# migoox/genome-downsampler

Measured on AMD Instinct MI355X. Metric: Mreads/s selected at target coverage M=100, higher is better.
Workload: dtype u32

## Files before the change

genome-downsampler_amd/csrc/api/context.inc.hip:

```cpp
namespace {

thread_local char g_err[512] = "";

int fail(int code, const char* fmt, ...) {
    va_list ap;
    va_start(ap, fmt);
    vsnprintf(g_err, sizeof(g_err), fmt, ap);
    va_end(ap);
    return code;
}

#define HIP_TRY(expr)                                                                      \
    do {                                                                                   \
        hipError_t _e = (expr);                                                            \
        if (_e != hipSuccess)                                                              \
            return fail(_e == hipErrorOutOfMemory ? QMCP_ENOMEM : QMCP_EHIP, "%s: %s (%s:%d)", \
                        #expr, hipGetErrorString(_e), __FILE__, __LINE__);                 \
    } while (0)

struct DevBuf {
    void* p = nullptr;
    size_t cap = 0;
};

enum Ev { EV_BEGIN = 0, EV_PREP, EV_SCAN, EV_SORT, EV_SWEEP, EV_MARK, EV_COUNT };

struct Problem {
    uint64_t n = 0;
    uint32_t n_contigs = 0;
    uint64_t ltot = 0;
    std::vector<uint64_t> poff;
};

struct SolveRun {
    const uint32_t* d_starts = nullptr;
    const uint32_t* d_ends = nullptr;
    const uint64_t* roff = nullptr;
    const uint32_t* lengths = nullptr;
    uint32_t n_contigs = 0, M = 0;
    uint64_t n64 = 0;
    uint64_t* d_mask = nullptr;
    Problem pr;
    qmcp_hip_stats local;
    bool trivial = false, head_done = false, may_rank = false, two_level = false, have_gstart = true;
    bool ranked_counted = false, wait_empty = false;
    bool pm = false;
    uint32_t range_shift = 0;
    uint32_t nu_filter = 0;
};

}

struct qmcp_hip_ctx {
    int device = 0;
    qmcp_hip_options opt = {};
    hipStream_t stream = nullptr;
    hipEvent_t ev[EV_COUNT] = {};
    hipEvent_t ev_in = nullptr;
    hipStream_t stream2 = nullptr;
    hipEvent_t ev_fork = nullptr;
    DevBuf roff, poff, stats, cstart, boff, ecnt, eoff, selend, spine, hist, spine2, hist2, specsnap, specflags;
    DevBuf keys[2], vals[2];
    DevBuf in_starts, in_ends, in_aux0, in_aux1, mask, cov, amp, next_head;
    DevBuf f_starts, f_ends, f_map, f_words, f_mask;
    DevBuf ranges;
    DevBuf rankamb;
    DevBuf pm_desc, pm_work;
    uint32_t nu_ell = 0;
    uint64_t nu_failed_n = 0, nu_failed_ltot = 0;
    uint32_t nu_failed_ell = 0, nu_failed_M = 0;
    uint64_t nu_need_n = 0, nu_need_ltot = 0;
    uint32_t nu_need_ell = 0, nu_need_M = 0, nu_need_rounds = 0;
    bool nu_deferred = false;
    DevBuf nu_exc, nu_nadj, nu_ce, nu_state, nu_sus, nu_ckpt, nu_prev;
    uint32_t* h_nu = nullptr;
    uint64_t* h_tables = nullptr;
    size_t h_tables_cap = 0;
    unsigned long long* h_scalars = nullptr;
    uint32_t* h_stage = nullptr;
    size_t h_stage_words = 0;
    uint64_t* h_mask = nullptr;
    size_t h_mask_words = 0;
    std::vector<hipEvent_t> stage_ev;
    std::vector<hipStream_t> stage_streams;
    std::vector<hipEvent_t> stage_done;
    bool pending = false;
    qmcp_hip_stats pend_stats;
    uint32_t pend_whole_contig_chains = 0;
    bool spiky_known = false, pend_spiky = false;
    uint64_t spiky_n = 0, spiky_ltot = 0;
    uint32_t spiky_empty = 0;
    uint64_t spec_hopeless_n = 0, spec_hopeless_ltot = 0;
    uint32_t spec_hopeless_M = 0;
    uint32_t pend_M = 0;
    DevBuf scalars;
    DevBuf segs;
    DevBuf rings;
    DevBuf kidx;
    DevBuf bc_key, bc_rec[2], bc_hist, bc_spine, bc_offs, bc_err, bc_len, bc_starts, bc_ends, bc_mask;
    DevBuf af_ids, af_ids_c, af_len, af_tab, af_err;
    DevBuf qc_words, qc_tab, qc_bare, qc_keys[2], qc_vals[2], qc_hist, qc_spine, qc_kb, qc_end, qc_head;
    DevBuf tg_ps, tg_pe, tg_off, tg_offw, tg_q, tg_tab;
    DevBuf dr_ev, dr_tab, dr_acc, dr_hist, dr_sums, dr_cnt;
    DevBuf dt_cnt, dt_runs;
    DevBuf ld_starts[2], ld_ends[2], ld_orig[2], ld_words, ld_spine, ld_offs[2], ld_levels, ld_mask0;
    DevBuf st_strata, st_rows;
    DevBuf dd_tab, dd_stat, dd_bare, dd_keys[2], dd_vals[2], dd_hist, dd_spine, dd_flag, dd_head, dd_cid, dd_surv, dd_words,
        dd_histo, dd_cs, dd_ce, dd_ci, dd_map, dd_maskc, dd_tags, dd_dupm;
    DevBuf pf_need, pf_tab, pf_stat;
    DevBuf pr_in, pr_rest, pr_words, pr_spine, pr_offs[2], pr_poff, pr_credit, pr_cspine, pr_starts, pr_ends, pr_orig,
        pr_mask, pr_need, pr_stat;
    uint64_t mask_reads = 0;
    DevBuf evpk, evlast;
    uint32_t last_iters = 0, last_blocks = 0;
    SolveRun run;
    uint32_t* h_head = nullptr;
    hipEvent_t ev_head = nullptr;
    hipEvent_t ev_done = nullptr;
    bool mixed_seen = false;
    bool sized = false;
    uint32_t grew_mid_solve = 0;
    int profiling = 0;
    size_t tables_count = 0;
    void* tables_dev_roff = nullptr;
    void* tables_dev_poff = nullptr;
    struct Span { const char* name; hipEvent_t a, b; };
    std::vector<Span> spans;
    std::vector<hipEvent_t> ev_pool;
    struct Acc { std::string name; uint64_t launches; double ms; };
    std::vector<Acc> acc;
};

namespace {

hipEvent_t pool_event(qmcp_hip_ctx* c) {
    if (!c->ev_pool.empty()) {
        hipEvent_t e = c->ev_pool.back();
        c->ev_pool.pop_back();
        return e;
    }
    hipEvent_t e = nullptr;
    if (hipEventCreate(&e) != hipSuccess) return nullptr;
    return e;
}

struct KernelSpan {
    qmcp_hip_ctx* c;
    hipEvent_t a = nullptr, b = nullptr;
    const char* name;
    hipStream_t st;
    KernelSpan(qmcp_hip_ctx* ctx, const char* nm, hipStream_t stream = nullptr)
        : c(ctx), name(nm), st(stream ? stream : ctx->stream) {
        if (!c->profiling || !nm) return;
        if (c->profiling == 2 && std::strncmp(nm, "k_sweep", 7) != 0) return;
        a = pool_event(c);
        b = pool_event(c);
        if (a) (void)hipEventRecord(a, st);
    }
    ~KernelSpan() {
        if (!c->profiling || !a || !b) return;
        (void)hipEventRecord(b, st);
        c->spans.push_back({name, a, b});
    }
};

void collect_spans(qmcp_hip_ctx* c) {
    for (auto& sp : c->spans) {
        float ms = 0.f;
        if (hipEventElapsedTime(&ms, sp.a, sp.b) == hipSuccess) {
            bool found = false;
            for (auto& a : c->acc)
                if (a.name == sp.name) { a.launches++; a.ms += ms; found = true; break; }
            if (!found) c->acc.push_back({sp.name, 1, ms});
        }
        c->ev_pool.push_back(sp.a);
        c->ev_pool.push_back(sp.b);
    }
    c->spans.clear();
}

int ensure(qmcp_hip_ctx* c, DevBuf& b, size_t bytes) {
    if (bytes == 0) bytes = 16;
    if (b.cap >= bytes) return QMCP_OK;
    if (b.p) {
        if (c->sized) c->grew_mid_solve++;
        if (c->stream) HIP_TRY(hipStreamSynchronize(c->stream));
        if (c->stream2) HIP_TRY(hipStreamSynchronize(c->stream2));
        HIP_TRY(hipFree(b.p));
        b.p = nullptr;
        b.cap = 0;
    }
    HIP_TRY(hipMalloc(&b.p, bytes));
    b.cap = bytes;
    return QMCP_OK;
}

#define TRY(expr)                      \
    do {                               \
        int _rc = (expr);              \
        if (_rc != QMCP_OK) return _rc; \
    } while (0)

uint32_t bit_width(uint32_t v) { return v == 0 ? 0u : 32u - (uint32_t)__builtin_clz(v); }

int check_problem(const uint64_t* roff, const uint32_t* lengths, uint32_t n_contigs, uint64_t n,
                  Problem& pr) {
    if (!roff || !lengths || n_contigs == 0) return fail(QMCP_EINVAL, "contig tables missing or n_contigs == 0");
    if (roff[0] != 0 || roff[n_contigs] != n)
        return fail(QMCP_EINVAL, "contig_read_offsets must start at 0 and end at n_reads");
    pr.poff.assign((size_t)n_contigs + 1, 0);
    for (uint32_t c = 0; c < n_contigs; ++c) {
        if (roff[c + 1] < roff[c]) return fail(QMCP_EINVAL, "contig_read_offsets not monotone at %u", c);
        pr.poff[c + 1] = pr.poff[c] + lengths[c];
    }
    pr.n = n;
    pr.n_contigs = n_contigs;
    pr.ltot = pr.poff[n_contigs];
    if (n > (1ull << 30)) return fail(QMCP_ERANGE, "n_reads %llu exceeds 2^30 per call", (unsigned long long)n);
    if (pr.ltot > (1ull << 31) - 2)
        return fail(QMCP_ERANGE, "total contig length %llu exceeds 2^31-2", (unsigned long long)pr.ltot);
    return QMCP_OK;
}

int upload_tables(qmcp_hip_ctx* c, const uint64_t* roff, const Problem& pr) {
    const size_t count = (size_t)pr.n_contigs + 1;
    const size_t bytes = count * sizeof(uint64_t);
    TRY(ensure(c, c->roff, bytes));
    TRY(ensure(c, c->poff, bytes));
    if (c->h_tables_cap < 2 * count) {
        if (c->h_tables) HIP_TRY(hipHostFree(c->h_tables));
        c->h_tables = nullptr;
        HIP_TRY(hipHostMalloc((void**)&c->h_tables, 2 * bytes, hipHostMallocDefault));
        c->h_tables_cap = 2 * count;
    }
    if (c->tables_count == count && c->tables_dev_roff == c->roff.p && c->tables_dev_poff == c->poff.p &&
        std::memcmp(c->h_tables, roff, bytes) == 0 &&
        std::memcmp(c->h_tables + count, pr.poff.data(), bytes) == 0)
        return QMCP_OK;
    std::memcpy(c->h_tables, roff, bytes);
    std::memcpy(c->h_tables + count, pr.poff.data(), bytes);
    c->tables_count = count;
    c->tables_dev_roff = c->roff.p;
    c->tables_dev_poff = c->poff.p;
    HIP_TRY(hipMemcpyAsync(c->roff.p, c->h_tables, bytes, hipMemcpyHostToDevice, c->stream));
    HIP_TRY(hipMemcpyAsync(c->poff.p, c->h_tables + count, bytes, hipMemcpyHostToDevice, c->stream));
    return QMCP_OK;
}

int run_prepare(qmcp_hip_ctx* c, const uint32_t* d_starts, const uint32_t* d_ends,
                const Problem& pr, const uint64_t* d_keep_mask, bool want_keys, bool want_counts,
                bool want_part_hist, uint32_t part_shift, uint32_t* d_global_digit_hist,
                uint32_t host_stats[3]) {
    const uint32_t n = (uint32_t)pr.n;
    TRY(ensure(c, c->stats, 4 * sizeof(uint32_t)));
    if (want_counts) TRY(ensure(c, c->cstart, ((size_t)pr.ltot + 1) * sizeof(uint32_t)));
    if (want_keys) TRY(ensure(c, c->vals[1], (size_t)n * sizeof(uint32_t)));
    const uint32_t init[4] = {0xFFFFFFFFu, 0u, 0u, 0u};
    HIP_TRY(hipMemcpyAsync(c->stats.p, init, sizeof(init), hipMemcpyHostToDevice, c->stream));
    if (want_counts)
        HIP_TRY(hipMemsetAsync(c->cstart.p, 0, ((size_t)pr.ltot + 1) * sizeof(uint32_t), c->stream));
    {
        KernelSpan sp(c, "k_prepare");
        qmcp::launch_prepare(c->stream, d_starts, d_ends, n, (const uint64_t*)c->roff.p,
                             (const uint64_t*)c->poff.p, pr.n_contigs, d_keep_mask,
                             want_keys ? (uint32_t*)c->vals[1].p : nullptr,
                             want_counts ? (uint32_t*)c->cstart.p : nullptr, (uint32_t*)c->stats.p,
                             part_shift, want_part_hist ? (uint32_t*)c->hist2.p : nullptr, nullptr,
                             d_global_digit_hist, nullptr);
    }
    HIP_TRY(hipGetLastError());
    HIP_TRY(hipMemcpyAsync(host_stats, c->stats.p, 3 * sizeof(uint32_t), hipMemcpyDeviceToHost,
                           c->stream));
    HIP_TRY(hipStreamSynchronize(c->stream));
    if (host_stats[2] != 0)
        return fail(QMCP_EREAD, "a read has start > end or end >= its contig length");
    return QMCP_OK;
}

int scan_counts(qmcp_hip_ctx* c, DevBuf& counts, DevBuf& out, uint32_t ltot) {
    TRY(ensure(c, out, ((size_t)ltot + 1) * sizeof(uint32_t)));
    TRY(ensure(c, c->spine, (size_t)qmcp::scan_spine_entries(ltot) * sizeof(uint32_t) + 16));
    {
        KernelSpan sp(c, "scan_positions(3 kernels)");
        qmcp::launch_exclusive_scan(c->stream, (const uint32_t*)counts.p, ltot, (uint32_t*)out.p,
                                    (uint32_t*)c->spine.p, true);
    }
    HIP_TRY(hipGetLastError());
    return QMCP_OK;
}

constexpr uint64_t kRankBalance = 24;
static uint32_t rank_min_reads(const qmcp_hip_ctx* c) { return c->opt.rank_min_reads ? c->opt.rank_min_reads : (1u << 17); }

float elapsed(hipEvent_t a, hipEvent_t b) {
    float ms = 0.f;
    if (hipEventElapsedTime(&ms, a, b) != hipSuccess) return 0.f;
    return ms;
}
```

genome-downsampler_amd/csrc/api/near_uniform_route.inc.hip:

```cpp
constexpr uint32_t kNuRunInsApart = 2;
int near_uniform_tail(qmcp_hip_ctx* c, uint32_t min_span, uint32_t max_span, uint32_t max_load, uint32_t* d_iters, bool& done) {
    done = false;
    SolveRun& run = c->run;
    const Problem& pr = run.pr;
    qmcp_hip_stats& local = run.local;
    const uint32_t n = (uint32_t)pr.n, ltot = (uint32_t)pr.ltot, n_contigs = run.n_contigs, M = run.M;
    local.near_uniform_giveup = QMCP_NU_GIVEUP_NOT_TRIED;
    if (c->opt.near_uniform < 0) return QMCP_OK;
    const uint32_t ell = max_span;
    uint32_t longest = 0;
    for (uint32_t k = 0; k < n_contigs; ++k) longest = run.lengths[k] > longest ? run.lengths[k] : longest;
    const qmcp::NearUniformPlan plan = qmcp::plan_near_uniform(c->opt, n, ell, min_span, ltot, n_contigs, longest, M, run.may_rank);
    const bool stretches = plan.stretches, speculate = plan.speculate;
    const bool dbg = c->opt.near_uniform_debug == 1;
    if (dbg) fprintf(stderr, "[near] pm %d may_rank %d ell %u ev %d depth %.2f min_span %u filter %u\n", (int)run.pm,
                     (int)run.may_rank, ell, (int)qmcp::sweep_uniform_ev_supported(ell, M), plan.depth, min_span, run.nu_filter);
    if (!plan.tried) return QMCP_OK;
    if (c->nu_failed_n == run.n64 && c->nu_failed_ltot == pr.ltot && c->nu_failed_ell == ell && c->nu_failed_M == M) {
        local.near_uniform_giveup = QMCP_NU_GIVEUP_REMEMBERED;
        c->nu_ell = 0;
        return QMCP_OK;
    }
    hipStream_t st = c->stream;
    const uint32_t cap = nu_cap_for(n);
    uint32_t n_exc = 0;
    uint32_t* d_stats = (uint32_t*)c->stats.p;
    if (run.nu_filter == ell) {
        n_exc = c->h_head[5];
        if (c->h_head[6] != 0) { c->nu_ell = 0; local.near_uniform_giveup = QMCP_NU_GIVEUP_TOO_MANY; return QMCP_OK; }
    } else {
        TRY(ensure_near_uniform(c, n, ltot, n_contigs));
        HIP_TRY(hipMemsetAsync(d_stats + 7, 0, sizeof(uint32_t), st));
        qmcp::launch_nu_count_span(st, run.d_starts, run.d_ends, n, ell, d_stats + 7);
        HIP_TRY(hipMemcpyAsync(c->h_nu, d_stats + 7, sizeof(uint32_t), hipMemcpyDeviceToHost, st));
        HIP_TRY(hipStreamSynchronize(st));
        n_exc = n - c->h_nu[0];
        if (dbg) fprintf(stderr, "[near] reads of span %u: %u of %u, list holds %u\n", ell, c->h_nu[0], n, cap);
        if (n_exc > n / 10u) {
            c->nu_ell = 0;
            local.near_uniform_giveup = n_exc > n - n / 10u ? QMCP_NU_GIVEUP_LONGER_READS : QMCP_NU_GIVEUP_TOO_MANY;
            return QMCP_OK;
        }
        c->nu_ell = ell;
        if (run.pm) TRY(queue_pm_head(c, st, ell));
        else TRY(queue_rm_head(c, st, ell, true));
        uint32_t* d_max_load = (uint32_t*)c->ranges.p + 65540;
        HIP_TRY(hipMemcpyAsync(c->h_nu, d_max_load, sizeof(uint32_t), hipMemcpyDeviceToHost, st));
        HIP_TRY(hipMemcpyAsync(c->h_nu + 1, d_stats + 4, 2 * sizeof(uint32_t), hipMemcpyDeviceToHost, st));
        HIP_TRY(hipStreamSynchronize(st));
        max_load = c->h_nu[0];
        if (c->h_nu[1] != n_exc || c->h_nu[2] != 0) { c->nu_ell = 0; local.near_uniform_giveup = QMCP_NU_GIVEUP_TOO_MANY; return QMCP_OK; }
    }
    local.near_uniform_exceptions = n_exc;
    if (n_exc == 0 || n_exc > n / 10u || (uint64_t)max_load * kRankBalance > (uint64_t)n) {
        if (n_exc > n / 10u) c->nu_ell = 0;
        local.near_uniform_giveup = n_exc > n / 10u ? QMCP_NU_GIVEUP_TOO_MANY : n_exc == 0 ? QMCP_NU_GIVEUP_NOT_TRIED : QMCP_NU_GIVEUP_HEAVY_RANGE;
        return QMCP_OK;
    }
    if (!stretches) {
        TRY(ensure(c, c->evpk, qmcp::sweep_ev_pack_bytes(ltot, ell, n_contigs + 768)));
        TRY(ensure(c, c->evlast, qmcp::sweep_ev_last_bytes(ltot, ell, n_contigs + 768)));
    }
    const uint32_t* boff = (const uint32_t*)c->boff.p;
    const uint64_t* poff = (const uint64_t*)c->poff.p;
    uint32_t* selend = (uint32_t*)c->selend.p;
    uint32_t* exc = (uint32_t*)c->nu_exc.p;
    int32_t* nadj = (int32_t*)c->nu_nadj.p;
    uint32_t* state = (uint32_t*)c->nu_state.p;
    unsigned long long* viol_key = (unsigned long long*)((char*)c->nu_state.p + 64);
    uint32_t* viol_idx = (uint32_t*)(viol_key + n_contigs);
    uint32_t* sweep_from[2] = {viol_idx + n_contigs, viol_idx + 2 * (size_t)n_contigs};
    if (!stretches) TRY(ensure(c, c->nu_ckpt, qmcp::sweep_ev_ckpt_bytes(ltot, ell, n_contigs + 768)));
    HIP_TRY(hipMemsetAsync(sweep_from[0], 0, (size_t)n_contigs * sizeof(uint32_t), st));
    HIP_TRY(hipEventRecord(c->ev[EV_SCAN], st));
    HIP_TRY(hipEventRecord(c->ev[EV_SORT], st));
    {
        KernelSpan sp(c, "near-uniform setup (exception coverage, need, pre-selection)");
        qmcp::launch_nu_setup(st, exc, cap, n_exc, d_stats + 6, boff, ltot, ell, M, (uint32_t*)c->nu_ce.p, (uint32_t*)c->spine.p,
                              nadj, state);
    }
    const uint32_t* seg = nullptr;
    uint32_t n_seg_max = 0;
    const uint32_t windows = plan.windows, burn_blocks = plan.burn_blocks;
    if (windows != 0) {
        KernelSpan sp(c, "k_find_cuts", st);
        seg = qmcp::launch_sweep_segments(st, boff, nullptr, poff, n_contigs, ltot, ell, M, windows, (uint32_t*)c->segs.p,
                                          (const uint32_t*)c->nu_ce.p);
        n_seg_max = n_contigs + windows;
    }
    uint32_t* marks[2] = {(uint32_t*)((char*)c->nu_sus.p + qmcp::nu_suspect_bytes(nu_suspects_for(n))), nullptr};
    const uint32_t mw = nu_marks_words(n_contigs);
    marks[1] = marks[0] + mw;
    uint32_t* fine[2] = {marks[1] + mw, marks[1] + 2 * (size_t)mw};
    uint32_t* dirty[2] = {fine[1] + mw, nullptr};
    dirty[1] = dirty[0] + qmcp::nu_cells_bytes() / sizeof(uint32_t);
    if (stretches) HIP_TRY(hipMemsetAsync(dirty[0], 0, 2 * qmcp::nu_cells_bytes(), st));
    const uint32_t* seg_fine = speculate ? (const uint32_t*)c->segs.p + windows + (1 + 5 * ((size_t)n_contigs + windows)) : nullptr;
    if (c->opt.near_uniform_debug == 2) seg_fine = nullptr;
    uint32_t rounds = 0;
    bool settled = false;
    const uint32_t budget = nu_round_budget(c, run.lengths, n_contigs);
    const bool defer = !dbg && c->opt.near_uniform_rounds == 0 && c->nu_need_rounds != 0 && c->nu_need_rounds <= 8 &&
                       c->nu_need_n == run.n64 && c->nu_need_ltot == pr.ltot && c->nu_need_ell == ell && c->nu_need_M == M &&
                       run.nu_filter == ell;
    while (rounds < budget && !settled) {
        const uint32_t batch = 2u;
        for (uint32_t r = 0; r < batch; ++r) {
            ++rounds;
            if (stretches) {
                if (speculate) {
                    TRY(speculative_sweep(
                        c, st, n_contigs, ltot, windows, ell, ell, burn_blocks, kNuRunInsApart, seg, "k_sweep_uniform_gen",
                        [&](const uint32_t* table, uint32_t* run_in_out, const uint32_t* redo_in) {
                            return qmcp::launch_sweep_uniform_gen(st, boff, poff, n_contigs, ell, M, ltot, selend, d_iters, table,
                                                                  n_seg_max, run_in_out, redo_in, nadj,
                                                                  (table == seg_fine && rounds > 1) ? fine[0] : nullptr);
                        },
                        [&](const uint32_t* table, uint32_t* mismatches, const uint32_t* redo_in, uint32_t* redo_out) {
                            qmcp::launch_spec_verify(st, table, n_seg_max, ell, selend, (const uint32_t*)c->cstart.p, mismatches,
                                                     redo_in, redo_out, (table == seg_fine && rounds > 1) ? fine[0] : nullptr);
                        },
                        rounds == 1 ? nullptr : marks[0]));
                } else {
                    KernelSpan sp(c, "k_sweep_uniform_gen", st);
                    if (!qmcp::launch_sweep_uniform_gen(st, boff, poff, n_contigs, ell, M, ltot, selend, d_iters, seg, n_seg_max,
                                                        nullptr, (seg != nullptr && rounds > 1) ? marks[0] : nullptr, nadj))
                        return fail(QMCP_ERANGE, "near-uniform route: span %u not supported", ell);
                }
            } else {
            {
                KernelSpan sp(c, "k_sweep_pack", st);
                qmcp::launch_sweep_ev_pack(st, boff, poff, n_contigs, ell, M, ltot, nullptr, 0, (uint32_t*)c->evpk.p, nadj, sweep_from[0]);
            }
            {
                KernelSpan sp(c, "k_sweep_uniform_ev", st);
                qmcp::launch_sweep_ev_chain(st, boff, poff, n_contigs, ell, M, ltot, nullptr, 0, (const uint32_t*)c->evpk.p,
                                            (uint32_t*)c->cstart.p, (uint32_t*)c->evlast.p, d_iters, nadj, (uint32_t*)c->nu_ckpt.p,
                                            sweep_from[0]);
            }
            {
                KernelSpan sp(c, "k_sweep_expand", st);
                qmcp::launch_sweep_ev_expand(st, boff, poff, n_contigs, ell, M, ltot, nullptr, 0, (const uint32_t*)c->cstart.p,
                                             (const uint32_t*)c->evlast.p, selend, sweep_from[0]);
            }
            }
            {
                KernelSpan sp(c, "near-uniform round (verify, replay, select, apply)");
                qmcp::launch_nu_round(st, exc, cap, n_exc, d_stats + 6, rounds == 1, boff, selend, nadj, (const uint32_t*)c->nu_ce.p, poff, n_contigs, ell, M,
                                      (uint2*)c->nu_sus.p, nu_suspects_for(n), state, viol_key, viol_idx, sweep_from[0], sweep_from[1],
                                      ltot, (uint32_t*)c->spine.p, stretches ? seg : nullptr, n_seg_max, marks[1],
                                      stretches ? (uint32_t*)c->nu_prev.p : nullptr, dirty[0], dirty[1], seg_fine, fine[1]);
                std::swap(sweep_from[0], sweep_from[1]);
                std::swap(marks[0], marks[1]);
                std::swap(fine[0], fine[1]);
                std::swap(dirty[0], dirty[1]);
            }
        }
        HIP_TRY(hipGetLastError());
        if (defer && rounds < c->nu_need_rounds) continue;
        HIP_TRY(hipMemcpyAsync(c->h_nu, state, 8 * sizeof(uint32_t), hipMemcpyDeviceToHost, st));
        if (defer) break;
        HIP_TRY(hipStreamSynchronize(st));
        if (dbg) {
            uint32_t more[8];
            (void)hipMemcpy(more, state + 8, sizeof(more), hipMemcpyDeviceToHost);
            fprintf(stderr, "[near] open question: s %u u1 %u S(u1-1) %u C(u1-1) %u b %u c0 %u\n", more[0], more[1], more[2], more[3], more[4], more[5]);
            fprintf(stderr, "[near] after %u rounds: last round selected %u, flags %u (read %u), selected in all %u, suspects %u, rounds that selected %u; next sweeps from block",
                    rounds, c->h_nu[1], c->h_nu[2], c->h_nu[5], c->h_nu[3], c->h_nu[4], c->h_nu[6]);
            std::vector<uint32_t> from(n_contigs);
            (void)hipMemcpy(from.data(), sweep_from[0], (size_t)n_contigs * sizeof(uint32_t), hipMemcpyDeviceToHost);
            for (uint32_t k = 0; k < n_contigs && k < 16; ++k) fprintf(stderr, " %d", (int)from[k]);
            fprintf(stderr, "\n");
        }
        if (c->h_nu[2] != 0) break;
        settled = c->h_nu[1] == 0;
    }
    c->nu_deferred = defer;
    if (defer) {
        settled = true;
    } else if (settled) {
        c->nu_need_n = run.n64; c->nu_need_ltot = pr.ltot; c->nu_need_ell = ell; c->nu_need_M = M;
        c->nu_need_rounds = rounds;
        rounds = c->h_nu[6] + 1;
    }
    local.near_uniform_rounds = rounds;
    local.near_uniform_selected = defer ? 0u : c->h_nu[3];
    if (!settled) {
        c->nu_need_rounds = 0;
        local.near_uniform_giveup = c->h_nu[2] != 0 ? QMCP_NU_GIVEUP_UNMODELLED : QMCP_NU_GIVEUP_BUDGET;
        c->nu_ell = 0;
        c->nu_failed_n = run.n64; c->nu_failed_ltot = pr.ltot; c->nu_failed_ell = ell; c->nu_failed_M = M;
        return QMCP_OK;
    }
    local.near_uniform_giveup = QMCP_NU_GIVEUP_NONE;
    HIP_TRY(hipEventRecord(c->ev[EV_SWEEP], st));
    if (run.pm) {
        queue_pm_rank(c, st, nullptr, nullptr, 0);
    } else {
        KernelSpan sp(c, "k_rank_mark");
        qmcp::launch_rank_mark(st, (const uint16_t*)c->keys[0].p, (const uint32_t*)c->vals[0].p, (const uint32_t*)c->ranges.p,
                               run.range_shift, ltot, boff, selend, (unsigned long long*)run.d_mask,
                               (unsigned long long*)c->scalars.p, c->rankamb.p,
                               qmcp::rank_scratch_by_records(run.range_shift, ltot, n));
    }
    {
        KernelSpan sp(c, "k_nu_mark_selected");
        qmcp::launch_nu_mark_selected(st, exc, cap, n_exc, d_stats + 6, (unsigned long long*)run.d_mask,
                                      (unsigned long long*)c->scalars.p);
    }
    HIP_TRY(hipGetLastError());
    done = true;
    return QMCP_OK;
}
```

genome-downsampler_amd/csrc/api/solve_head.inc.hip:

```cpp
int queue_rm_head(qmcp_hip_ctx* c, hipStream_t s1, uint32_t filter, bool clear_mask);
int queue_pm_head(qmcp_hip_ctx* c, hipStream_t st, uint32_t filter);

bool pm_route_ok(const qmcp_hip_ctx* c, const uint64_t* roff, const Problem& pr, uint32_t shift) {
    if (c->opt.pass_major < 0) return false;
    const uint32_t n = (uint32_t)pr.n, ltot = (uint32_t)pr.ltot;
    if ((uint64_t)qmcp::pm_slots(n, ltot, shift) >= (1ull << 31)) return false;
    if (c->opt.pass_major > 0) return true;
    double slots = 0.0;
    for (uint32_t k = 0; k < pr.n_contigs; ++k) {
        const uint64_t reads = roff[k + 1] - roff[k];
        if (reads == 0 || pr.poff[k + 1] == pr.poff[k]) continue;
        const double ranges = (double)(((pr.poff[k + 1] - 1) >> shift) - (pr.poff[k] >> shift) + 1);
        const double passes = (double)reads / (double)qmcp::pm_pass() < 1.0 ? 1.0 : (double)reads / (double)qmcp::pm_pass();
        const double slice = (double)reads / (passes * ranges);
        slots += passes * ranges * std::ceil(slice / 64.0);
    }
    return slots <= 1.3 * ((double)n / 64.0);
}
int enqueue_head(qmcp_hip_ctx* c, const uint32_t* d_starts, const uint32_t* d_ends,
                 const uint64_t* roff, const uint32_t* lengths, uint32_t n_contigs, uint64_t n64,
                 uint32_t M, uint64_t* d_mask) {
    if (c->pending) return fail(QMCP_EINVAL, "a solve is already pending on this context (call qmcp_hip_solve_end)");
    c->pend_spiky = false;
    if (!c->h_scalars) HIP_TRY(hipHostMalloc((void**)&c->h_scalars, 16 * sizeof(unsigned long long), hipHostMallocDefault));
    SolveRun& run = c->run;
    run = SolveRun();
    run.d_starts = d_starts; run.d_ends = d_ends; run.roff = roff; run.lengths = lengths;
    run.n_contigs = n_contigs; run.n64 = n64; run.M = M; run.d_mask = d_mask;
    Problem& pr = run.pr;
    TRY(check_problem(roff, lengths, n_contigs, n64, pr));
    const uint32_t n = (uint32_t)pr.n;
    const uint32_t ltot = (uint32_t)pr.ltot;
    const size_t mask_words = (size_t)((n64 + 63) / 64);
    qmcp_hip_stats& local = run.local;
    std::memset(&local, 0, sizeof(local));
    local.n_reads = n64;
    local.n_contigs = n_contigs;
    local.total_length = pr.ltot;
    if (n == 0 || ltot == 0) {
        if (mask_words) HIP_TRY(hipMemsetAsync(d_mask, 0, mask_words * sizeof(uint64_t), c->stream));
        if (n != 0) return fail(QMCP_EREAD, "reads given for zero-length contigs");
        run.trivial = true;
        HIP_TRY(hipEventRecord(c->ev[EV_BEGIN], c->stream));
        return QMCP_OK;
    }
    c->sized = false;
    {
        const uint32_t tiles_seg = qmcp::seg_tile_bound(n);
        const uint32_t spine_a = qmcp::scan_spine_entries(256u * tiles_seg);
        const uint32_t spine_b = qmcp::scan_spine_entries(ltot + 1) + 1;
        TRY(ensure(c, c->spine, (size_t)(spine_a > spine_b ? spine_a : spine_b) * sizeof(uint32_t) + 16));
        TRY(ensure(c, c->hist, (size_t)256 * tiles_seg * sizeof(uint32_t)));
        const bool may_pm = n >= rank_min_reads(c) && qmcp::range_path_supported(ltot) && !qmcp::range_path_two_level(ltot) &&
                            pm_route_ok(c, roff, pr, qmcp::range_shift_for(ltot));
        const size_t pm_bytes = may_pm ? qmcp::pm_slots(n, ltot, qmcp::range_shift_for(ltot)) * sizeof(uint16_t) : 0;
        TRY(ensure(c, c->keys[0], std::max((size_t)n * sizeof(uint64_t), pm_bytes)));
        TRY(ensure(c, c->keys[1], std::max((size_t)n * sizeof(uint64_t), pm_bytes)));
        if (may_pm) {
            const size_t groups = pm_bytes / (64 * sizeof(uint16_t));
            TRY(ensure(c, c->pm_desc, groups * sizeof(uint32_t)));
            TRY(ensure(c, c->pm_work, 1024 * sizeof(uint32_t)));
        }
        TRY(ensure(c, c->vals[0], (size_t)n * sizeof(uint32_t)));
        TRY(ensure(c, c->vals[1], (size_t)n * sizeof(uint32_t)));
        TRY(ensure(c, c->spine2, (size_t)(spine_a > spine_b ? spine_a : spine_b) * sizeof(uint32_t) + 16));
        TRY(ensure(c, c->hist2, ((size_t)256 * qmcp::part_pass_pitch(n) + 4) * sizeof(uint32_t)));
        TRY(ensure(c, c->cstart, ((size_t)ltot + 8) * sizeof(uint32_t)));
        TRY(ensure(c, c->boff, ((size_t)ltot + 1) * sizeof(uint32_t)));
        TRY(ensure(c, c->selend, ((size_t)ltot + 8) * sizeof(uint32_t)));
        TRY(ensure(c, c->scalars, 64));
        TRY(ensure(c, c->segs, qmcp::sweep_segment_words(n_contigs < 256 ? n_contigs : 0, qmcp::kMaxSweepWindows) * sizeof(uint32_t)));
        TRY(ensure(c, c->specflags, 2 * 4096 * sizeof(uint32_t)));
        TRY(ensure(c, c->specsnap, qmcp::spec_snap_bytes(4096)));
        TRY(ensure(c, c->ranges, (65537 + 7 + 771 + 5) * sizeof(uint32_t)));
        if (n >= rank_min_reads(c) && qmcp::range_path_supported(ltot))
            TRY(ensure(c, c->rankamb, qmcp::rank_scratch_bytes(qmcp::range_shift_for(ltot), ltot, n)));
        TRY(ensure(c, c->stats, 12 * sizeof(uint32_t)));
        if (c->nu_ell != 0 || c->mixed_seen) TRY(ensure_near_uniform(c, n, ltot, n_contigs));
        if (c->mixed_seen || !(n >= rank_min_reads(c) && qmcp::range_path_supported(ltot))) {
            TRY(ensure(c, c->ecnt, ((size_t)ltot + 1) * sizeof(uint32_t)));
            TRY(ensure(c, c->eoff, ((size_t)ltot + 1) * sizeof(uint32_t)));
            TRY(ensure(c, c->next_head, ((size_t)n + 2) * sizeof(uint32_t)));
            TRY(ensure(c, c->spine, (size_t)(qmcp::scan_spine_entries(n + 1) + 1) * sizeof(uint32_t) + 16));
        }
    }
    c->grew_mid_solve = 0;
    HIP_TRY(hipEventRecord(c->ev[EV_BEGIN], c->stream));
    TRY(upload_tables(c, roff, pr));
    c->sized = true;

    uint32_t* const hs = c->h_head;
    run.range_shift = qmcp::range_shift_for(ltot);
    run.may_rank = n >= rank_min_reads(c) && qmcp::range_path_supported(ltot);
    const uint32_t range_shift = run.range_shift;
    uint32_t* d_range_start = (uint32_t*)c->ranges.p;
    uint32_t* d_max_load = d_range_start + 65540;
    uint32_t* d_seg_tables = d_range_start + 65544;
    run.two_level = qmcp::range_path_two_level(ltot);
    const bool two_level = run.two_level;
    hs[3] = 0;
    hs[4] = 0xFFFFFFFFu;
    run.have_gstart = true;
    if (!run.may_rank) {
        HIP_TRY(hipMemsetAsync(d_mask, 0, mask_words * sizeof(uint64_t), c->stream));
        uint32_t hs3[3];
        TRY(run_prepare(c, d_starts, d_ends, pr, nullptr, true, false, false, range_shift, nullptr, hs3));
        hs[0] = hs3[0]; hs[1] = hs3[1]; hs[2] = hs3[2];
        HIP_TRY(hipEventRecord(c->ev[EV_PREP], c->stream));
    } else {
        run.have_gstart = false;
        hipStream_t s1 = c->stream;
        static const uint32_t init[8] = {0xFFFFFFFFu, 0u, 0u, 0u, 0u, 0u, 0u, 0u};
        HIP_TRY(hipMemcpyAsync(c->stats.p, init, sizeof(init), hipMemcpyHostToDevice, s1));
        run.pm = !two_level && pm_route_ok(c, roff, pr, range_shift);
        run.nu_filter = c->nu_ell;
        hs[5] = hs[6] = 0;
        if (run.pm) {
            TRY(queue_pm_head(c, s1, run.nu_filter));
        } else {
            TRY(queue_rm_head(c, s1, run.nu_filter, true));
        }
        HIP_TRY(hipGetLastError());
        HIP_TRY(hipEventRecord(c->ev_head, s1));
        HIP_TRY(hipStreamWaitEvent(c->stream2, c->ev_fork, 0));
        HIP_TRY(hipMemcpyAsync(hs, c->stats.p, 3 * sizeof(uint32_t), hipMemcpyDeviceToHost, c->stream2));
        HIP_TRY(hipMemcpyAsync(hs + 3, d_max_load, sizeof(uint32_t), hipMemcpyDeviceToHost, c->stream2));
        if (run.nu_filter) HIP_TRY(hipMemcpyAsync(hs + 5, (uint32_t*)c->stats.p + 4, 2 * sizeof(uint32_t), hipMemcpyDeviceToHost, c->stream2));
        if (c->spiky_known && c->spiky_n == n64 && c->spiky_ltot == pr.ltot) {
            hs[4] = c->spiky_empty;
        } else {
            HIP_TRY(hipMemcpyAsync(hs + 4, (uint32_t*)c->stats.p + 3, sizeof(uint32_t), hipMemcpyDeviceToHost, s1));
            run.wait_empty = true;
        }
        run.ranked_counted = true;
    }
    run.head_done = true;
    return QMCP_OK;
}

int queue_rm_head(qmcp_hip_ctx* c, hipStream_t s1, uint32_t filter, bool clear_mask) {
    SolveRun& run = c->run;
    const uint32_t n = (uint32_t)run.pr.n, ltot = (uint32_t)run.pr.ltot, n_contigs = run.n_contigs;
    const uint32_t range_shift = run.range_shift;
    const bool two_level = run.two_level;
    uint32_t* d_range_start = (uint32_t*)c->ranges.p;
    uint32_t* d_max_load = d_range_start + 65540;
    uint32_t* d_seg_tables = d_range_start + 65544;
    static const uint32_t zeros[4] = {0u, 0u, 0u, 0u};
    HIP_TRY(hipMemcpyAsync((uint32_t*)c->stats.p + 3, zeros, sizeof(zeros), hipMemcpyHostToDevice, s1));
    uint32_t* exc = filter ? (uint32_t*)c->nu_exc.p : nullptr;
    const uint32_t cap = nu_cap_for(n);
    uint32_t* exc_cnt = filter ? qmcp::nu_exc_counts(exc, cap) : nullptr;
    if (filter) HIP_TRY(hipMemsetAsync(exc_cnt, 0, ((size_t)cap / 128 + 4) * sizeof(uint32_t), s1));
    {
        KernelSpan sp(c, "k_prepare");
        qmcp::launch_prepare(s1, run.d_starts, run.d_ends, n, (const uint64_t*)c->roff.p,
                             (const uint64_t*)c->poff.p, n_contigs, nullptr, nullptr, nullptr,
                             (uint32_t*)c->stats.p, two_level ? range_shift + 8 : range_shift,
                             (uint32_t*)c->hist2.p, nullptr, nullptr,
                             clear_mask ? (unsigned long long*)run.d_mask : nullptr,
                             filter, exc, cap, exc_cnt);
    }
    HIP_TRY(hipGetLastError());
    HIP_TRY(hipEventRecord(c->ev[EV_PREP], s1));
    {
        KernelSpan sp(c, "scan_radix_hist(3 kernels)");
        qmcp::launch_exclusive_scan(s1, (const uint32_t*)c->hist2.p, 256u * qmcp::part_pass_pitch(n),
                                    (uint32_t*)c->hist2.p, (uint32_t*)c->spine2.p, true);
    }
    if (!two_level) {
        KernelSpan sp(c, "k_range_partition");
        qmcp::launch_range_partition(s1, nullptr, run.d_starts, (const uint64_t*)c->roff.p,
                                     (const uint64_t*)c->poff.p, n_contigs, n, range_shift,
                                     (const uint32_t*)c->hist2.p, (uint16_t*)c->keys[0].p,
                                     (uint32_t*)c->vals[0].p, d_range_start, d_max_load, run.d_ends, filter);
    } else {
        {
            KernelSpan sp(c, "k_range_partition(level 1)");
            qmcp::launch_partition_level1(s1, run.d_starts, (const uint64_t*)c->roff.p,
                                          (const uint64_t*)c->poff.p, n_contigs, n, range_shift + 8,
                                          (const uint32_t*)c->hist2.p, c->keys[1].p, d_seg_tables, d_max_load,
                                          run.d_ends, filter);
        }
        KernelSpan sp(c, "partition level 2 (tables, hist, scan, scatter)");
        qmcp::launch_partition_level2(s1, c->keys[1].p, n, range_shift, d_seg_tables, (uint32_t*)c->hist.p,
                                      (uint32_t*)c->spine.p, (uint16_t*)c->keys[0].p,
                                      (uint32_t*)c->vals[0].p, d_range_start, d_max_load);
    }
    HIP_TRY(hipEventRecord(c->ev_fork, s1));
    {
        KernelSpan sp(c, "k_range_offsets");
        qmcp::launch_range_offsets(s1, (const uint16_t*)c->keys[0].p, d_range_start, range_shift, ltot,
                                   (uint32_t*)c->boff.p, (uint32_t*)c->stats.p + 3);
    }
    HIP_TRY(hipGetLastError());
    run.nu_filter = filter;
    return QMCP_OK;
}

int queue_pm_head(qmcp_hip_ctx* c, hipStream_t st, uint32_t filter) {
    SolveRun& run = c->run;
    const uint32_t n = (uint32_t)run.pr.n, ltot = (uint32_t)run.pr.ltot, n_contigs = run.n_contigs;
    uint32_t* d_stats = (uint32_t*)c->stats.p;
    static const uint32_t zeros[4] = {0u, 0u, 0u, 0u};
    HIP_TRY(hipMemcpyAsync(d_stats + 3, zeros, sizeof(zeros), hipMemcpyHostToDevice, st));
    uint32_t* d_range_start = (uint32_t*)c->ranges.p;
    uint32_t* d_max_load = d_range_start + 65540;
    {
        KernelSpan sp(c, "k_pm_prepare_sort", st);
        qmcp::launch_pm_prepare_sort(st, run.d_starts, run.d_ends, n, (const uint64_t*)c->roff.p, (const uint64_t*)c->poff.p,
                                     n_contigs, run.range_shift, ltot, (uint16_t*)c->keys[0].p, (uint16_t*)c->keys[1].p,
                                     (uint32_t*)c->hist2.p, (uint32_t*)c->hist.p,
                                     (uint32_t*)c->pm_work.p, d_stats, (unsigned long long*)run.d_mask, filter,
                                     filter ? (uint32_t*)c->nu_exc.p : nullptr, nu_cap_for(n),
                                     filter ? qmcp::nu_exc_counts((uint32_t*)c->nu_exc.p, nu_cap_for(n)) : nullptr);
    }
    HIP_TRY(hipGetLastError());
    HIP_TRY(hipEventRecord(c->ev[EV_PREP], st));
    {
        KernelSpan sp(c, "scan_radix_hist(3 kernels)", st);
        qmcp::launch_exclusive_scan(st, (const uint32_t*)c->hist2.p, 256u * qmcp::pm_pitch(n), (uint32_t*)c->hist2.p,
                                    (uint32_t*)c->spine2.p, true);
    }
    {
        KernelSpan sp(c, "k_pm_descr + k_pm_range_table", st);
        qmcp::launch_pm_descr(st, (const uint32_t*)c->hist2.p, (const uint32_t*)c->hist.p, n, ltot, run.range_shift,
                              (uint32_t*)c->pm_desc.p, (uint32_t*)c->pm_work.p, d_range_start, d_max_load);
    }
    HIP_TRY(hipEventRecord(c->ev_fork, st));
    {
        KernelSpan sp(c, "k_pm_offsets", st);
        qmcp::launch_pm_offsets(st, (const uint16_t*)c->keys[0].p, (const uint32_t*)c->pm_desc.p, (const uint32_t*)c->hist2.p, n,
                                d_range_start, run.range_shift, ltot, (uint32_t*)c->boff.p, d_stats + 3);
    }
    HIP_TRY(hipGetLastError());
    run.nu_filter = filter;
    return QMCP_OK;
}

void queue_pm_rank(qmcp_hip_ctx* c, hipStream_t st, const uint32_t* ev_sev, const uint32_t* ev_lastns, uint32_t ell) {
    SolveRun& run = c->run;
    const uint32_t n = (uint32_t)run.pr.n, ltot = (uint32_t)run.pr.ltot;
    const bool by_records = qmcp::rank_scratch_by_records(run.range_shift, ltot, n);
    const uint16_t* keys16 = (const uint16_t*)c->keys[0].p;
    const uint16_t* idx16 = (const uint16_t*)c->keys[1].p;
    const uint32_t* desc = (const uint32_t*)c->pm_desc.p;
    const uint32_t* Tp = (const uint32_t*)c->hist2.p;
    const uint32_t* range_start = (const uint32_t*)c->ranges.p;
    uint32_t* amb_count = (uint32_t*)c->pm_work.p + 512;
    unsigned long long* kept_total = (unsigned long long*)c->scalars.p;
    {
        KernelSpan sp(c, "k_pm_walk", st);
        qmcp::launch_pm_walk(st, keys16, idx16, desc, Tp, n, range_start, run.range_shift, ltot, (const uint32_t*)c->boff.p,
                             (const uint32_t*)c->selend.p, (unsigned long long*)run.d_mask, kept_total, c->rankamb.p, by_records,
                             amb_count, ev_sev, ev_lastns, (const uint64_t*)c->poff.p, run.n_contigs, ell);
    }
    KernelSpan sp(c, "k_pm_settle", st);
    qmcp::launch_pm_settle(st, keys16, idx16, desc, Tp, n, range_start, run.range_shift, ltot, c->rankamb.p, by_records,
                           amb_count, (unsigned long long*)run.d_mask, kept_total);
}
```

genome-downsampler_amd/csrc/api/solve_tail.inc.hip:

```cpp
int enqueue_tail(qmcp_hip_ctx* c) {
    SolveRun& run = c->run;
    const Problem& pr = run.pr;
    qmcp_hip_stats& local = run.local;
    const uint32_t n = (uint32_t)pr.n, ltot = (uint32_t)pr.ltot, n_contigs = run.n_contigs, M = run.M;
    const uint64_t n64 = run.n64;
    const uint32_t *d_starts = run.d_starts, *d_ends = run.d_ends;
    uint64_t* const d_mask = run.d_mask;
    const uint64_t* roff = run.roff;
    const uint32_t* lengths = run.lengths;
    if (run.trivial) {
        for (int i = EV_PREP; i <= EV_MARK; ++i) HIP_TRY(hipEventRecord(c->ev[i], c->stream));
        for (int i = 0; i < 8; ++i) c->h_scalars[i] = 0;
        c->pend_stats = local;
        c->pend_whole_contig_chains = 0;
        c->pending = true;
        return QMCP_OK;
    }
    const uint32_t range_shift = run.range_shift;
    const bool may_rank = run.may_rank;
    uint32_t* d_range_start = (uint32_t*)c->ranges.p;
    const uint32_t* hs = c->h_head;
    bool have_gstart = run.have_gstart;
    const bool ranked_counted = run.ranked_counted;
    if (may_rank) {
        HIP_TRY(hipStreamSynchronize(c->stream2));
        if (run.wait_empty) HIP_TRY(hipStreamSynchronize(c->stream));
        if (hs[2] != 0) {
            (void)hipStreamSynchronize(c->stream);
            return fail(QMCP_EREAD, "a read has start > end or end >= its contig length");
        }
    }
    const uint32_t max_load = hs[3];
    const uint32_t empty_positions = hs[4];
    const uint32_t min_span = hs[0], max_span = hs[1];
    local.min_span = min_span;
    local.max_span = max_span;
    const bool uniform = (min_span == max_span) && max_span <= qmcp::kMaxUniformSpan;
    if (!uniform && max_span > qmcp::kMaxGeneralSpan)
        return fail(QMCP_ERANGE, "mixed-span reads with span %u > %u are not supported by this build",
                    max_span, qmcp::kMaxGeneralSpan);
    local.path = uniform ? QMCP_PATH_UNIFORM : QMCP_PATH_GENERAL;
    if (uniform)
        for (uint32_t k = 0; k < n_contigs; ++k)
            if (roff[k + 1] - roff[k] >= (1ull << 28))
                return fail(QMCP_ERANGE, "contig %u holds %llu reads; the block sweep handles < 2^28 per contig",
                            k, (unsigned long long)(roff[k + 1] - roff[k]));

    const uint32_t pos_bits = bit_width(ltot - 1) == 0 ? 1u : bit_width(ltot - 1);
    uint32_t span_bits = 0;
    bool wide = false;
    const uint32_t* d_gstart = (const uint32_t*)c->vals[1].p;
    const uint32_t* d_key32 = d_gstart;
    auto need_gstart = [&]() {
        if (have_gstart) return;
        KernelSpan sp(c, "k_gstart");
        qmcp::launch_gstart(c->stream, d_starts, n, (const uint64_t*)c->roff.p, (const uint64_t*)c->poff.p,
                            n_contigs, (uint32_t*)c->vals[1].p);
        have_gstart = true;
    };
    bool sweep_done = false, ranked = false;
    uint32_t* d_iters = (uint32_t*)((char*)c->scalars.p + 16);
    bool near_done = false;
    uint32_t max_load_now = max_load;
    if (uniform && run.nu_filter != 0 && run.nu_filter != max_span) {
        c->nu_ell = 0;
        if (run.pm) TRY(queue_pm_head(c, c->stream, 0));
        else TRY(queue_rm_head(c, c->stream, 0, true));
        HIP_TRY(hipMemcpyAsync(c->h_nu, (uint32_t*)c->ranges.p + 65540, sizeof(uint32_t), hipMemcpyDeviceToHost, c->stream));
        HIP_TRY(hipStreamSynchronize(c->stream));
        max_load_now = c->h_nu[0];
    }
    if (!uniform) c->mixed_seen = true;
    if (!uniform && max_span <= qmcp::kMaxUniformSpan) {
        HIP_TRY(hipMemsetAsync(c->scalars.p, 0, 64, c->stream));
        TRY(near_uniform_tail(c, min_span, max_span, max_load, d_iters, near_done));
        if (near_done) {
            local.path = QMCP_PATH_NEAR_UNIFORM;
            sweep_done = ranked = true;
        }
    }
    if (!uniform && !near_done) {
        need_gstart();
        span_bits = bit_width(max_span - min_span);
        wide = pos_bits + span_bits > 32;
        c->mixed_seen = true;
        TRY(ensure(c, c->ecnt, ((size_t)ltot + 1) * sizeof(uint32_t)));
        TRY(ensure(c, c->eoff, ((size_t)ltot + 1) * sizeof(uint32_t)));
        HIP_TRY(hipMemsetAsync(c->ecnt.p, 0, ((size_t)ltot + 1) * sizeof(uint32_t), c->stream));
        void* key_dst = wide ? c->keys[0].p : c->vals[0].p;
        {
            KernelSpan sp(c, "k_general_keys");
            qmcp::launch_general_keys(c->stream, wide, d_gstart, d_starts, d_ends, n, span_bits,
                                      max_span, nullptr, key_dst, (uint32_t*)c->ecnt.p, ltot + 1);
        }
        HIP_TRY(hipGetLastError());
        TRY(scan_counts(c, c->ecnt, c->eoff, ltot));
        d_key32 = (const uint32_t*)c->vals[0].p;
    }
    if (!near_done) HIP_TRY(hipEventRecord(c->ev[EV_SCAN], c->stream));
    bool mixed_whole_contigs = false;
    if (!near_done) HIP_TRY(hipMemsetAsync(c->scalars.p, 0, 64, c->stream));
    if (uniform && may_rank) {
        hipStream_t s1 = c->stream;
        HIP_TRY(hipGetLastError());
        HIP_TRY(hipEventRecord(c->ev[EV_SORT], s1));
        ranked = (uint64_t)max_load_now * kRankBalance <= (uint64_t)n;
        if (c->opt.force_sort_route) ranked = false;
        bool expand_left_out = ranked && run.pm && !c->opt.keep_expand;
        TRY(launch_uniform_sweep(c, s1, n, ltot, n_contigs, max_span, M, d_iters, empty_positions, &expand_left_out));
        HIP_TRY(hipGetLastError());
        HIP_TRY(hipEventRecord(c->ev[EV_SWEEP], s1));
        sweep_done = true;
        if (ranked && run.pm) {
            queue_pm_rank(c, s1, expand_left_out ? (const uint32_t*)c->cstart.p : nullptr, (const uint32_t*)c->evlast.p, max_span);
            HIP_TRY(hipGetLastError());
        } else if (ranked) {
            KernelSpan sp(c, "k_rank_mark");
            qmcp::launch_rank_mark(s1, (const uint16_t*)c->keys[0].p, (const uint32_t*)c->vals[0].p,
                                   d_range_start, range_shift, ltot,
                                   (const uint32_t*)c->boff.p, (const uint32_t*)c->selend.p,
                                   (unsigned long long*)d_mask, (unsigned long long*)c->scalars.p,
                                   c->rankamb.p, qmcp::rank_scratch_by_records(range_shift, ltot, n));
            HIP_TRY(hipGetLastError());
        }
    }

    const uint32_t key_bits = pos_bits + span_bits;
    const uint32_t passes = (key_bits + 7) / 8;
    local.sort_passes = ranked ? 1u : passes;
    int kin = 0, vin = 0;
    if (!ranked && uniform) need_gstart();
    if (ranked) {
    } else if (!wide) {
        TRY(radix_sort_records(c, c->stream, d_key32, n, passes, (uint32_t*)c->hist.p, (uint32_t*)c->spine.p, c->keys,
                               {"k_radix_hist_rec", "scan_radix_hist(3 kernels)", "k_radix_scatter_rec"}, &kin));
    } else {
        WideBufs wb;
        TRY(radix_sort_wide(c, c->stream, n, passes, (uint32_t*)c->hist.p, (uint32_t*)c->spine.p, c->keys, c->vals,
                            {"k_radix_hist", "scan_radix_hist(3 kernels)", "k_radix_scatter"}, &wb));
        kin = wb.k;
        vin = wb.v;
    }
    if (!sweep_done) {
    HIP_TRY(hipMemsetAsync(c->boff.p, 0xFF, ((size_t)ltot + 1) * sizeof(uint32_t), c->stream));
    {
        KernelSpan sp(c, "k_bucket_heads");
        qmcp::launch_bucket_heads(c->stream, wide, c->keys[kin].p, (const uint32_t*)c->vals[vin].p, n,
                                  span_bits, ltot, (uint32_t*)c->boff.p);
    }
    {
        KernelSpan sp(c, "reverse_min_scan(3 kernels)");
        qmcp::launch_reverse_min_scan(c->stream, (uint32_t*)c->boff.p, ltot + 1, (uint32_t*)c->spine.p);
    }
    }
    HIP_TRY(hipGetLastError());
    if (!sweep_done) HIP_TRY(hipEventRecord(c->ev[EV_SORT], c->stream));

    if (sweep_done) {
    } else if (uniform) {
        TRY(launch_uniform_sweep(c, c->stream, n, ltot, n_contigs, max_span, M, d_iters, empty_positions));
    } else {
        uint32_t ring = 64;
        while (ring <= max_span) ring <<= 1;
        const uint32_t* seg = nullptr;
        uint32_t n_seg_max = 0;
        const bool in_regs = max_span + 64 <= 512 && !c->opt.mixed_sweep_in_lds;
        qmcp::MixedSweepPlan plan = qmcp::plan_mixed_sweep(
            c->opt, n, max_span, ltot, n_contigs, M, in_regs,
            c->spec_hopeless_n == n64 && c->spec_hopeless_ltot == pr.ltot && c->spec_hopeless_M == M);
        const uint32_t windows = plan.windows;
        if (windows != 0) {
            KernelSpan sp(c, "k_find_cuts");
            seg = qmcp::launch_sweep_segments(c->stream, (const uint32_t*)c->boff.p, (const uint32_t*)c->eoff.p,
                                              (const uint64_t*)c->poff.p, n_contigs, ltot, max_span, M, windows,
                                              (uint32_t*)c->segs.p);
            n_seg_max = n_contigs + windows;
            HIP_TRY(hipMemcpyAsync(d_iters + 2, seg, sizeof(uint32_t), hipMemcpyDeviceToDevice, c->stream));
        }
        mixed_whole_contigs = seg == nullptr;
        if (max_span <= qmcp::kMaxCachedSpan) {
            ring = 64;
            while (ring < max_span + 64) ring <<= 1;
            TRY(ensure(c, c->next_head, ((size_t)n + 2) * sizeof(uint32_t)));
            TRY(ensure(c, c->spine, (size_t)(qmcp::scan_spine_entries(n + 1) + 1) * sizeof(uint32_t) + 16));
            {
                KernelSpan sp(c, "k_group_heads");
                qmcp::launch_group_heads(c->stream, wide, c->keys[kin].p, n, (uint32_t*)c->next_head.p);
            }
            {
                KernelSpan sp(c, "reverse_min_scan(3 kernels)");
                qmcp::launch_reverse_min_scan(c->stream, (uint32_t*)c->next_head.p, n + 1,
                                              (uint32_t*)c->spine.p);
            }
            if (plan.sample_span_mode) {
                uint32_t* d_share = (uint32_t*)c->stats.p + 6;
                qmcp::launch_span_mode_share(c->stream, d_starts, d_ends, n, d_share);
                uint32_t share[3] = {0, 0, 0};
                HIP_TRY(hipMemcpyAsync(share, d_share, sizeof(share), hipMemcpyDeviceToHost, c->stream));
                HIP_TRY(hipStreamSynchronize(c->stream));
                uint32_t longest = 0;
                for (uint32_t k = 0; k < n_contigs; ++k) longest = lengths[k] > longest ? lengths[k] : longest;
                plan = qmcp::refine_mixed_with_span_sample(c->opt, plan, share, longest);
            }
            const bool speculate = plan.speculate;
            if (speculate) {
                TRY(ensure(c, c->specsnap, qmcp::spec_snap_bytes(n_seg_max)));
                const void* sorted = c->keys[kin].p;
                TRY(speculative_sweep(
                    c, c->stream, n_contigs, ltot, windows, max_span, plan.round_to, plan.burn_blocks, plan.run_ins_apart, seg,
                    "k_sweep_general_reg",
                    [&](const uint32_t* table, uint32_t* out_odd, const uint32_t* redo_in) {
                        return qmcp::launch_sweep_general_reg(c->stream, wide, (const uint32_t*)c->boff.p, (const uint32_t*)c->eoff.p,
                                                              sorted, (const uint32_t*)c->next_head.p, (const uint64_t*)c->poff.p,
                                                              n_contigs, span_bits, max_span, M, (uint32_t*)c->selend.p, table,
                                                              n_seg_max, out_odd, redo_in, (uint32_t*)c->specsnap.p);
                    },
                    [&](const uint32_t* table, uint32_t* mismatches, const uint32_t* redo_in, uint32_t* redo_out) {
                        qmcp::launch_spec_verify_merge_mixed(c->stream, table, n_seg_max, max_span, (uint32_t*)c->selend.p,
                                                             (const uint32_t*)c->cstart.p, (const uint32_t*)c->specsnap.p,
                                                             mismatches, redo_in, redo_out);
                    }));
                HIP_TRY(hipMemcpyAsync(d_iters + 2, (uint32_t*)c->segs.p + windows + (1 + 5 * (size_t)n_seg_max), sizeof(uint32_t),
                                       hipMemcpyDeviceToDevice, c->stream));
            }
            if (!speculate) {
                KernelSpan sp(c, in_regs ? "k_sweep_general_reg" : "k_sweep_general_cached");
                if (!in_regs ||
                    !qmcp::launch_sweep_general_reg(c->stream, wide, (const uint32_t*)c->boff.p,
                                                    (const uint32_t*)c->eoff.p, c->keys[kin].p,
                                                    (const uint32_t*)c->next_head.p, (const uint64_t*)c->poff.p,
                                                    n_contigs, span_bits, max_span, M, (uint32_t*)c->selend.p, seg,
                                                    n_seg_max))
                    qmcp::launch_sweep_general_cached(c->stream, wide, (const uint32_t*)c->boff.p,
                                                      (const uint32_t*)c->eoff.p, c->keys[kin].p,
                                                      (const uint32_t*)c->next_head.p, (const uint64_t*)c->poff.p,
                                                      n_contigs, span_bits, max_span, M,
                                                      (uint32_t*)c->selend.p, ring, seg, n_seg_max);
            }
        } else {
            uint32_t* g_rings = nullptr;
            if (max_span > qmcp::kMaxLdsRingSpan) {
                const size_t n_wg = seg ? n_seg_max : n_contigs;
                TRY(ensure(c, c->rings, n_wg * 2 * (size_t)ring * sizeof(uint32_t)));
                g_rings = (uint32_t*)c->rings.p;
            }
            KernelSpan sp(c, "k_sweep_general");
            qmcp::launch_sweep_general(c->stream, wide, (const uint32_t*)c->boff.p,
                                       (const uint32_t*)c->eoff.p, c->keys[kin].p,
                                       (const uint64_t*)c->poff.p, n_contigs, span_bits, max_span, M,
                                       (uint32_t*)c->selend.p, ring, seg, n_seg_max, g_rings);
        }
    }
    HIP_TRY(hipGetLastError());
    if (!sweep_done) HIP_TRY(hipEventRecord(c->ev[EV_SWEEP], c->stream));

    if (!ranked) {
        KernelSpan sp(c, "k_mark");
        qmcp::launch_mark(c->stream, wide, c->keys[kin].p, (const uint32_t*)c->vals[vin].p, ltot,
                          (const uint32_t*)c->boff.p, (const uint32_t*)c->selend.p, d_mask,
                          (unsigned long long*)c->scalars.p);
    }
    HIP_TRY(hipGetLastError());
    HIP_TRY(hipEventRecord(c->ev[EV_MARK], c->stream));
    HIP_TRY(hipMemcpyAsync(c->h_scalars, c->scalars.p, 7 * sizeof(unsigned long long), hipMemcpyDeviceToHost,
                           c->stream));
    c->pend_spiky = ranked_counted;
    if (ranked_counted) {
        HIP_TRY(hipMemcpyAsync(c->h_scalars + 7, (uint32_t*)c->stats.p + 3, sizeof(uint32_t), hipMemcpyDeviceToHost, c->stream));
        c->spiky_n = n64;
        c->spiky_ltot = pr.ltot;
    }
    c->pend_stats = local;
    c->pend_M = M;
    c->pend_whole_contig_chains = 0;
    if (mixed_whole_contigs)
        for (uint32_t k = 0; k < n_contigs; ++k) c->pend_whole_contig_chains += lengths[k] != 0 ? 1u : 0u;
    c->pending = true;
    return QMCP_OK;
}

int solve_enqueue(qmcp_hip_ctx* c, const uint32_t* d_starts, const uint32_t* d_ends, const uint64_t* roff,
                  const uint32_t* lengths, uint32_t n_contigs, uint64_t n64, uint32_t M, uint64_t* d_mask);
int collect_one(qmcp_hip_ctx* c, qmcp_hip_stats* st) {
    if (!c->pending) return fail(QMCP_EINVAL, "no solve is pending on this context");
    c->pending = false;
    HIP_TRY(hipStreamSynchronize(c->stream));
    if (c->nu_deferred) {
        c->nu_deferred = false;
        if (c->h_nu[2] != 0 || c->h_nu[1] != 0) {
            c->nu_need_rounds = 0;
            const SolveRun r = c->run;
            const size_t count = (size_t)r.n_contigs + 1;
            std::vector<uint64_t> roff(c->h_tables, c->h_tables + count);
            std::vector<uint32_t> lengths(r.n_contigs);
            for (uint32_t k = 0; k < r.n_contigs; ++k) lengths[k] = (uint32_t)(c->h_tables[count + k + 1] - c->h_tables[count + k]);
            TRY(solve_enqueue(c, r.d_starts, r.d_ends, roff.data(), lengths.data(), r.n_contigs, r.n64, r.M, r.d_mask));
            return collect_one(c, st);
        }
        c->pend_stats.near_uniform_rounds = c->h_nu[6] + 1;
        c->pend_stats.near_uniform_selected = c->h_nu[3];
    }
    collect_spans(c);
#ifdef QMCP_EV_STAMP
    if (c->scalars.p) {
        uint32_t raw[16];
        HIP_TRY(hipMemcpy(raw, c->scalars.p, sizeof(raw), hipMemcpyDeviceToHost));
        const uint32_t* it = raw + 4;
        fprintf(stderr, "[ev stamp] changed %u of %u blocks, stretches %u | x16 cycles: total %u general %u wait-for-ring %u slow-pieces %u (%u pieces) "
                        "failing rounds %u (%u rounds), blocks through the two scans %u\n",
                it[0], it[1], it[2], it[4], it[5], it[6], it[7], it[8], it[9], it[10], it[11]);
    }
#endif
    qmcp_hip_stats local = c->pend_stats;
    const unsigned long long* host_scalars = c->h_scalars;
    if (c->pend_spiky) {
        c->spiky_empty = (uint32_t)(c->h_scalars[7] & 0xFFFFFFFFull);
        c->spiky_known = true;
    }
    local.n_kept = host_scalars[0];
    c->last_iters = (uint32_t)(host_scalars[2] & 0xFFFFFFFFu);
    c->last_blocks = (uint32_t)(host_scalars[2] >> 32);
    local.sweep_blocks_changed = c->last_iters;
    local.sweep_blocks = c->last_blocks;
    local.sweep_stretches = (uint32_t)(host_scalars[3] & 0xFFFFFFFFu) + c->pend_whole_contig_chains;
    local.spec_mismatches = (uint32_t)(host_scalars[4] & 0xFFFFFFFFu);
    local.spec_boundaries = (uint32_t)(host_scalars[4] >> 32);
    local.spec_retry_mismatches = local.spec_mismatches ? (uint32_t)(host_scalars[5] & 0xFFFFFFFFu) : 0u;
    if (local.path == QMCP_PATH_GENERAL && local.spec_boundaries >= 4 && 2u * local.spec_mismatches > local.spec_boundaries &&
        c->opt.speculation_run_in == 0) {
        c->spec_hopeless_n = local.n_reads; c->spec_hopeless_ltot = local.total_length; c->spec_hopeless_M = c->pend_M;
    }
    local.ms_prepare = elapsed(c->ev[EV_BEGIN], c->ev[EV_PREP]);
    local.ms_scan = elapsed(c->ev[EV_PREP], c->ev[EV_SCAN]);
    local.ms_sort = elapsed(c->ev[EV_SCAN], c->ev[EV_SORT]);
    local.ms_sweep = elapsed(c->ev[EV_SORT], c->ev[EV_SWEEP]);
    local.ms_mark = elapsed(c->ev[EV_SWEEP], c->ev[EV_MARK]);
    local.ms_total = elapsed(c->ev[EV_BEGIN], c->ev[EV_MARK]);
    local.arena_grown_mid_solve = c->grew_mid_solve;
    if (st) *st = local;
    return QMCP_OK;
}

int solve_complete(qmcp_hip_ctx* c, qmcp_hip_stats* st) { return collect_one(c, st); }

void options_from_env(qmcp_hip_options& o) {
    auto num = [](const char* name) -> uint32_t { const char* e = std::getenv(name); return e ? (uint32_t)std::strtoul(e, nullptr, 10) : 0u; };
    auto flag = [](const char* name) -> int32_t { return std::getenv(name) != nullptr ? 1 : 0; };
    auto tri = [](const char* name) -> int32_t { const char* e = std::getenv(name); return !e ? 0 : e[0] == '1' ? 1 : e[0] == '0' ? -1 : 0; };
    o.pass_major = tri("QMCP_HIP_PM");
    if (const char* e = std::getenv("QMCP_HIP_SWEEP"))
        o.sweep = std::strcmp(e, "fast") == 0 ? QMCP_SWEEP_FAST : std::strcmp(e, "gen") == 0 ? QMCP_SWEEP_GENERAL
                  : std::strcmp(e, "ev") == 0 ? QMCP_SWEEP_EVENTS : QMCP_SWEEP_AUTO;
    o.cut_points = tri("QMCP_HIP_CUTS");
    o.speculation = tri("QMCP_HIP_SPEC");
    o.speculation_run_in = num("QMCP_HIP_SPEC_BURN");
    o.near_uniform = tri("QMCP_HIP_NEAR") < 0 ? -1 : 0;
    o.near_uniform_rounds = num("QMCP_HIP_NEAR_ROUNDS");
    if (const char* e = std::getenv("QMCP_HIP_NEAR_MIN_DEPTH")) o.near_uniform_min_depth = (float)std::strtod(e, nullptr);
    o.near_uniform_debug = flag("QMCP_HIP_NEAR_DEBUG");
    o.force_sort_route = flag("QMCP_HIP_NO_RANK");
    o.keep_expand = flag("QMCP_HIP_EXPAND");
    o.mixed_sweep_in_lds = flag("QMCP_HIP_GENERAL_LDS");
    o.rank_min_reads = num("QMCP_HIP_RANK_MIN");
    o.host_threads = num("QMCP_HIP_HOST_THREADS");
    o.copy_streams = num("QMCP_HIP_COPY_STREAMS");
    o.host_both_columns = flag("QMCP_HIP_HOST_BOTH_COLUMNS");
}

int create_ctx(int device, qmcp_hip_ctx** out_ctx) {
    if (!out_ctx) return fail(QMCP_EINVAL, "out_ctx is null");
    *out_ctx = nullptr;
    int n = 0;
    if (hipGetDeviceCount(&n) != hipSuccess || n <= 0) {
        (void)hipGetLastError();
        return fail(QMCP_ENODEVICE, "no HIP device available (quasi-mcp-hip has no CPU fallback)");
    }
    if (device < 0 || device >= n) return fail(QMCP_ENODEVICE, "device %d out of range [0,%d)", device, n);
    HIP_TRY(hipSetDevice(device));
    qmcp_hip_ctx* c = new (std::nothrow) qmcp_hip_ctx();
    if (!c) return fail(QMCP_ENOMEM, "host allocation failed");
    c->device = device;
    qmcp_hip_default_options(&c->opt);
    options_from_env(c->opt);
    hipError_t e = hipStreamCreateWithFlags(&c->stream, hipStreamNonBlocking);
    for (int i = 0; e == hipSuccess && i < EV_COUNT; ++i) e = hipEventCreate(&c->ev[i]);
    if (e == hipSuccess) e = hipEventCreateWithFlags(&c->ev_in, hipEventDisableTiming);
    if (e == hipSuccess) {
        int lo = 0, hi = 0;
        (void)hipDeviceGetStreamPriorityRange(&lo, &hi);
        e = hipStreamCreateWithPriority(&c->stream2, hipStreamNonBlocking, hi);
    }
    if (e == hipSuccess) e = hipEventCreateWithFlags(&c->ev_fork, hipEventDisableTiming);
    if (e == hipSuccess) e = hipEventCreateWithFlags(&c->ev_head, hipEventDisableTiming);
    if (e == hipSuccess) e = hipEventCreateWithFlags(&c->ev_done, hipEventDisableTiming);
    if (e == hipSuccess) e = hipHostMalloc((void**)&c->h_head, 8 * sizeof(uint32_t), hipHostMallocDefault);
    if (e != hipSuccess) {
        qmcp_hip_destroy(c);
        return fail(QMCP_EHIP, "context setup: %s", hipGetErrorString(e));
    }
    *out_ctx = c;
    return QMCP_OK;
}


int solve_enqueue(qmcp_hip_ctx* c, const uint32_t* d_starts, const uint32_t* d_ends,
                  const uint64_t* roff, const uint32_t* lengths, uint32_t n_contigs, uint64_t n64,
                  uint32_t M, uint64_t* d_mask) {
    if (c->pending) return fail(QMCP_EINVAL, "a solve is already pending on this context (call qmcp_hip_solve_end)");
    TRY(enqueue_head(c, d_starts, d_ends, roff, lengths, n_contigs, n64, M, d_mask));
    return enqueue_tail(c);
}

int solve_on_device(qmcp_hip_ctx* c, const uint32_t* d_starts, const uint32_t* d_ends,
                    const uint64_t* roff, const uint32_t* lengths, uint32_t n_contigs, uint64_t n64,
                    uint32_t M, uint64_t* d_mask, qmcp_hip_stats* st) {
    TRY(solve_enqueue(c, d_starts, d_ends, roff, lengths, n_contigs, n64, M, d_mask));
    return solve_complete(c, st);
}

int use_device(qmcp_hip_ctx* c, bool may_be_pending = false) {
    if (!c) return fail(QMCP_EINVAL, "null context");
    if (c->pending && !may_be_pending)
        return fail(QMCP_EINVAL, "a solve is pending on this context (call qmcp_hip_solve_end first)");
    HIP_TRY(hipSetDevice(c->device));
    return QMCP_OK;
}

int order_after(qmcp_hip_ctx* c, void* user_stream) {
    if ((hipStream_t)user_stream != c->stream) {
        HIP_TRY(hipEventRecord(c->ev_in, (hipStream_t)user_stream));
        HIP_TRY(hipStreamWaitEvent(c->stream, c->ev_in, 0));
    }
    return QMCP_OK;
}
```

genome-downsampler_amd/csrc/kernels/pass_major.inc.hip:

```cpp
static constexpr int kPmPass = 8192;
__host__ __device__ inline uint32_t pm_stride_of(uint32_t n_ranges) { return (uint32_t)kPmPass + 64u * n_ranges; }
static constexpr int kPmThreads = 512;
static constexpr int kPmWaves = kPmThreads / 64;
static constexpr int kPmPassesPerWg = 4;
static constexpr size_t kPmSortLds = ((size_t)kPmPass + kPmWaves * 256 + 2 * 256 + 16 + 2 * kPmPassesPerWg * 256 + kPmWaves * 3 * 128) * sizeof(uint32_t);
static constexpr uint32_t kPmExcPerWave = 128;

#ifndef QMCP_PM_MIN_WAVES
#define QMCP_PM_MIN_WAVES 4
#endif
__global__ __launch_bounds__(kPmThreads, QMCP_PM_MIN_WAVES) void k_pm_prepare_sort(
    const uint32_t* __restrict__ starts, const uint32_t* __restrict__ ends, uint32_t n,
    const uint64_t* __restrict__ contig_read_off, const uint64_t* __restrict__ contig_pos_off, uint32_t n_contigs,
    uint32_t shift, uint32_t stride ,
    uint16_t* __restrict__ keys16, uint16_t* __restrict__ idx16,
    uint32_t* __restrict__ cnt_tab, uint32_t* __restrict__ lst_tab, uint32_t pitch ,
    uint32_t* __restrict__ work ,
    uint32_t* __restrict__ stats, unsigned long long* __restrict__ zero_mask,
    uint32_t ell_reg, uint32_t* __restrict__ exc, uint32_t exc_cap, uint32_t* __restrict__ exc_cnt) {
    extern __shared__ uint32_t s_pm[];
    uint32_t* s_stage = s_pm;
    uint32_t* s_cnt = s_stage + kPmPass;
    uint32_t* s_gbase = s_cnt + kPmWaves * 256;
    uint32_t* s_pbase = s_gbase + 256;
    uint32_t* s_wave = s_pbase + 256;
    uint32_t* s_tabc = s_wave + 16;
    uint32_t* s_tabl = s_tabc + kPmPassesPerWg * 256;
    uint32_t* s_exc = s_tabl + kPmPassesPerWg * 256;
    if (blockIdx.x == 0 && threadIdx.x < 260) work[threadIdx.x] = 0;
    const int lane = threadIdx.x & 63, w = threadIdx.x >> 6;
    uint32_t mn = 0xFFFFFFFFu, mx = 0, bad = 0;
    auto contig_of = [&](uint32_t i) {
        uint32_t lo = 0, hi = n_contigs;
        while (hi - lo > 1) {
            const uint32_t mid = (lo + hi) >> 1;
            if (contig_read_off[mid] <= i) lo = mid; else hi = mid;
        }
        return lo;
    };
    for (int g = 0; g < kPmPassesPerWg; ++g) {
        const uint32_t P = blockIdx.x * kPmPassesPerWg + g;
        const uint64_t base64 = (uint64_t)P * kPmPass;
        if (base64 >= n) {
            if (threadIdx.x < 256) { s_tabc[g * 256 + threadIdx.x] = 0; s_tabl[g * 256 + threadIdx.x] = 0; }
            if (ell_reg != 0u && lane == 0 && P < pitch) exc_cnt[P * kPmWaves + w] = 0;
            continue;
        }
        const uint32_t base = (uint32_t)base64;
        const uint32_t count = min((uint32_t)kPmPass, n - base);
        const uint32_t wbase = base + w * (kSortItems * 64);
        Rec rec[kSortItems];
#pragma unroll
        for (int k = 0; k < kSortItems; ++k) {
            const uint32_t i = min(wbase + k * 64 + lane, n - 1);
            rec[k].key = starts[i];
            rec[k].val = ends[i];
        }
        for (int i = threadIdx.x; i < kPmWaves * 256; i += kPmThreads) s_cnt[i] = 0;
        if (zero_mask && threadIdx.x < 128 && P * 128u + threadIdx.x < (n + 63u) / 64u) zero_mask[P * 128u + threadIdx.x] = 0ull;
        const uint32_t c_first = n_contigs > 1 ? contig_of(base) : 0u;
        const uint32_t c_last = n_contigs > 1 ? contig_of(base + count - 1) : 0u;
        uint32_t match_bits;
        {
            const uint32_t d_lo = ((uint32_t)contig_pos_off[c_first] >> shift) & 255u;
            const uint32_t d_hi = ((uint32_t)contig_pos_off[c_last + 1] >> shift) & 255u;
            match_bits = d_hi >= d_lo ? 32u - (uint32_t)__builtin_clz((d_hi - d_lo) | 1u) : 8u;
            if (d_hi == d_lo) match_bits = 0;
        }
        uint32_t skip = 0;
        uint32_t filled = 0;
        typedef __attribute__((address_space(3))) uint32_t LdsWord;
        LdsWord* const mine = (LdsWord*)(s_exc + w * (3 * kPmExcPerWave));
        auto put_aside = [&, mine](int k, bool isx, uint32_t gs, uint32_t ge, uint32_t i) {
            const uint64_t m = __ballot(isx);
            if (m != 0ull) {
                const uint32_t slot = filled + __builtin_amdgcn_mbcnt_hi((uint32_t)(m >> 32), __builtin_amdgcn_mbcnt_lo((uint32_t)m, 0u));
                if (isx) {
                    skip |= 1u << k;
                    if (slot < kPmExcPerWave) { mine[3u * slot] = gs; mine[3u * slot + 1u] = ge; mine[3u * slot + 2u] = i; }
                    else nu_overflow_put(exc, exc_cap, stats, gs, ge, i);
                }
                filled += (uint32_t)__popcll(m);
            }
        };
        if (c_first == c_last) {
            const uint32_t p0 = (uint32_t)contig_pos_off[c_first];
            const uint32_t len = (uint32_t)contig_pos_off[c_first + 1] - p0;
            const uint32_t last = len ? len - 1u : 0u;
#pragma unroll
            for (int k = 0; k < kSortItems; ++k) {
                const uint32_t i = wbase + k * 64 + lane;
                const uint32_t s = rec[k].key, e = rec[k].val;
                bool isx = false;
                if (i < n) {
                    bad |= (s > e || e >= len) ? 1u : 0u;
                    const uint32_t span = e - s + 1;
                    mn = min(mn, span);
                    mx = max(mx, span);
                    isx = span != ell_reg;
                }
                rec[k].key = p0 + min(s, last);
                if (ell_reg != 0u) put_aside(k, isx, rec[k].key, p0 + min(e, last), i);
            }
        } else {
#pragma unroll
            for (int k = 0; k < kSortItems; ++k) {
                const uint32_t i = wbase + k * 64 + lane;
                bool isx = false;
                uint32_t ge = 0;
                if (i < n) {
                    const uint32_t cc = contig_of(i);
                    const uint32_t p0 = (uint32_t)contig_pos_off[cc];
                    const uint32_t len = (uint32_t)contig_pos_off[cc + 1] - p0;
                    const uint32_t s = rec[k].key, e = rec[k].val;
                    bad |= (s > e || e >= len) ? 1u : 0u;
                    const uint32_t span = e - s + 1;
                    mn = min(mn, span);
                    mx = max(mx, span);
                    rec[k].key = p0 + min(s, len ? len - 1u : 0u);
                    isx = span != ell_reg;
                    ge = p0 + min(e, len ? len - 1u : 0u);
                }
                if (ell_reg != 0u) put_aside(k, isx, rec[k].key, ge, i);
            }
        }
        __syncthreads();
        uint32_t rank[kSortItems];
        {
            uint32_t* const s_cnt_w = s_cnt + w * 256;
            const uint32_t bound = base + count;
            switch (match_bits) {
                case 0: part_rank_rounds<0>(rec, rank, wbase, bound, shift, lane, s_cnt_w, skip); break;
                case 1: part_rank_rounds<1>(rec, rank, wbase, bound, shift, lane, s_cnt_w, skip); break;
                case 2: part_rank_rounds<2>(rec, rank, wbase, bound, shift, lane, s_cnt_w, skip); break;
                case 3: part_rank_rounds<3>(rec, rank, wbase, bound, shift, lane, s_cnt_w, skip); break;
                case 4: part_rank_rounds<4>(rec, rank, wbase, bound, shift, lane, s_cnt_w, skip); break;
                case 5: part_rank_rounds<5>(rec, rank, wbase, bound, shift, lane, s_cnt_w, skip); break;
                case 6: part_rank_rounds<6>(rec, rank, wbase, bound, shift, lane, s_cnt_w, skip); break;
                case 7: part_rank_rounds<7>(rec, rank, wbase, bound, shift, lane, s_cnt_w, skip); break;
                default: part_rank_rounds<8>(rec, rank, wbase, bound, shift, lane, s_cnt_w, skip); break;
            }
        }
        __syncthreads();
        if (threadIdx.x < 256) {
            const uint32_t d = threadIdx.x;
            uint32_t tot = 0;
#pragma unroll
            for (int x = 0; x < kPmWaves; ++x) tot += s_cnt[x * 256 + d];
            const uint32_t ptot = (tot + 63u) & ~63u;
            const uint32_t inc = wave_incl_scan_add(tot);
            const uint32_t pinc = wave_incl_scan_add(ptot);
            if (lane == 63) { s_wave[w] = inc; s_wave[8 + w] = pinc; }
            s_gbase[d] = inc - tot;
            s_pbase[d] = pinc - ptot;
            s_tabc[g * 256 + d] = ptot;
            s_tabl[g * 256 + d] = tot << 16;
        }
        __syncthreads();
        if (threadIdx.x < 256) {
            const uint32_t d = threadIdx.x;
            uint32_t wave_base = 0, pwave_base = 0;
            for (int x = 0; x < w; ++x) { wave_base += s_wave[x]; pwave_base += s_wave[8 + x]; }
            const uint32_t tile_off = s_gbase[d] + wave_base;
            const uint32_t ptile_off = s_pbase[d] + pwave_base;
            uint32_t run = tile_off;
#pragma unroll
            for (int x = 0; x < kPmWaves; ++x) { const uint32_t cx = s_cnt[x * 256 + d]; s_cnt[x * 256 + d] = run; run += cx; }
            s_gbase[d] = tile_off;
            s_pbase[d] = ptile_off;
            s_tabl[g * 256 + d] |= ptile_off >> 6;
        }
        __syncthreads();
#pragma unroll
        for (int k = 0; k < kSortItems; ++k) {
            const uint32_t i = wbase + k * 64 + lane;
            if (i < n && !((skip >> k) & 1u)) {
                const uint32_t d = (rec[k].key >> shift) & 255u;
                const uint32_t local = (uint32_t)(w * (kSortItems * 64) + k * 64 + lane);
                s_stage[s_cnt[w * 256 + d] + rank[k]] = (rec[k].key & ((1u << shift) - 1u)) | (local << 16);
            }
        }
        __syncthreads();
        {
            const uint32_t my_d = (uint32_t)w + 8u * ((uint32_t)lane & 31u);
            const uint32_t my_tot = lane < 32 ? s_tabl[g * 256 + my_d] >> 16 : 0u;
            const uint32_t my_gb = s_gbase[my_d], my_pb = s_pbase[my_d];
            const bool upper = lane >= 32;
            const uint32_t hl = (uint32_t)lane & 31u;
            uint64_t todo = __ballot(my_tot != 0u);
            while (todo != 0ull) {
                const int l0 = __builtin_ctzll(todo);
                todo &= todo - 1ull;
                int l1 = l0;
                bool two = false;
                if (todo != 0ull) { l1 = __builtin_ctzll(todo); todo &= todo - 1ull; two = true; }
                const uint32_t cnt0 = (uint32_t)__builtin_amdgcn_readlane((int)my_tot, l0);
                const uint32_t cnt1 = two ? (uint32_t)__builtin_amdgcn_readlane((int)my_tot, l1) : 0u;
                const uint32_t cnt = upper ? cnt1 : cnt0;
                const uint32_t gb = upper ? (uint32_t)__builtin_amdgcn_readlane((int)my_gb, l1) : (uint32_t)__builtin_amdgcn_readlane((int)my_gb, l0);
                const uint32_t pb = upper ? (uint32_t)__builtin_amdgcn_readlane((int)my_pb, l1) : (uint32_t)__builtin_amdgcn_readlane((int)my_pb, l0);
                const size_t out0 = (size_t)P * stride + pb;
                const uint32_t most = max(cnt0, cnt1);
                for (uint32_t j0 = 0; j0 < most; j0 += 128u) {
                    const uint32_t j = j0 + 4u * hl;
                    if (j < cnt) {
                        const uint32_t v0 = s_stage[gb + j];
                        const uint32_t v1 = j + 1 < cnt ? s_stage[gb + j + 1] : 0u;
                        const uint32_t v2 = j + 2 < cnt ? s_stage[gb + j + 2] : 0u;
                        const uint32_t v3 = j + 3 < cnt ? s_stage[gb + j + 3] : 0u;
                        *reinterpret_cast<uint2*>(keys16 + out0 + j) = make_uint2((v0 & 0xFFFFu) | (v1 << 16), (v2 & 0xFFFFu) | (v3 << 16));
                        *reinterpret_cast<uint2*>(idx16 + out0 + j) = make_uint2((v0 >> 16) | (v1 & 0xFFFF0000u), (v2 >> 16) | (v3 & 0xFFFF0000u));
                    }
                }
            }
        }
        if (ell_reg != 0u) {
            const size_t slot0 = ((size_t)P * kPmWaves + w) * kPmExcPerWave;
            for (uint32_t r = (uint32_t)lane; r < min(filled, kPmExcPerWave); r += 64u) {
                exc[slot0 + r] = mine[3u * r];
                exc[exc_cap + slot0 + r] = mine[3u * r + 1u];
                exc[2 * (size_t)exc_cap + slot0 + r] = mine[3u * r + 2u];
            }
            if (lane == 0) {
                exc_cnt[P * kPmWaves + w] = min(filled, kPmExcPerWave);
            }
        }
        __syncthreads();
    }
    __syncthreads();
    if (threadIdx.x < 256) {
        const uint32_t P0 = blockIdx.x * kPmPassesPerWg;
        if (P0 < pitch) {
            uint4 a, b;
            a.x = s_tabc[threadIdx.x]; a.y = s_tabc[256 + threadIdx.x]; a.z = s_tabc[512 + threadIdx.x]; a.w = s_tabc[768 + threadIdx.x];
            b.x = s_tabl[threadIdx.x]; b.y = s_tabl[256 + threadIdx.x]; b.z = s_tabl[512 + threadIdx.x]; b.w = s_tabl[768 + threadIdx.x];
            *reinterpret_cast<uint4*>(cnt_tab + (size_t)threadIdx.x * pitch + P0) = a;
            *reinterpret_cast<uint4*>(lst_tab + (size_t)threadIdx.x * pitch + P0) = b;
        }
    }

    __shared__ uint32_t s_red[3][kPmWaves];
    mn = wave_min_u32(mn);
    mx = wave_max_u32(mx);
    bad = wave_max_u32(bad);
    if (lane == 0) { s_red[0][w] = mn; s_red[1][w] = mx; s_red[2][w] = bad; }
    __syncthreads();
    if (threadIdx.x == 0) {
        for (int x = 1; x < kPmWaves; ++x) { mn = min(mn, s_red[0][x]); mx = max(mx, s_red[1][x]); bad |= s_red[2][x]; }
        if (mn < __hip_atomic_load(&stats[0], __ATOMIC_RELAXED, __HIP_MEMORY_SCOPE_AGENT)) atomicMin(&stats[0], mn);
        if (mx > __hip_atomic_load(&stats[1], __ATOMIC_RELAXED, __HIP_MEMORY_SCOPE_AGENT)) atomicMax(&stats[1], mx);
        if (bad) atomicOr(&stats[2], 1u);
    }
}

static constexpr uint32_t kPmWorkWords = 260;
static constexpr uint32_t kPmDescrY = 8;

struct PmSlot { uint32_t slot0, nv, pass; };
template <bool kVector>
__device__ __forceinline__ PmSlot pm_unpack(uint32_t dsc, bool has, uint32_t stride) {
    PmSlot s;
    s.pass = dsc >> 15;
    s.slot0 = has ? (kVector ? __umul24(s.pass, stride) : s.pass * stride) + (((dsc >> 6) & 511u) << 6) : 0u;
    s.nv = has ? (dsc & 63u) + 1u : 0u;
    return s;
}

__global__ __launch_bounds__(256) void k_pm_descr(const uint32_t* __restrict__ Tp, const uint32_t* __restrict__ lstw,
                                                  uint32_t pitch, uint32_t n_groups ,
                                                  uint32_t* __restrict__ desc, uint32_t* __restrict__ work) {
    __shared__ uint32_t s_red[4];
    const uint32_t d = blockIdx.x;
    const uint32_t per = (pitch + gridDim.y - 1u) / gridDim.y;
    const uint32_t P_end = min(pitch, (blockIdx.y + 1u) * per);
    uint32_t mine = 0;
    for (uint32_t P0 = blockIdx.y * per + threadIdx.x; P0 < P_end; P0 += 4u * 256u) {
        uint32_t w[4], t[4];
#pragma unroll
        for (int u = 0; u < 4; ++u) {
            const uint32_t P = min(P0 + (uint32_t)u * 256u, P_end - 1u);
            w[u] = lstw[(size_t)d * pitch + P];
            t[u] = Tp[(size_t)d * pitch + P];
        }
#pragma unroll
        for (int u = 0; u < 4; ++u) {
            const uint32_t P = P0 + (uint32_t)u * 256u;
            const uint32_t cnt = P < P_end ? w[u] >> 16 : 0u;
            if (cnt == 0u) continue;
            mine += cnt;
            const uint32_t g = t[u] >> 6;
            const uint32_t n_ws = (cnt + 63u) >> 6;
            for (uint32_t j = 0; j < n_ws; ++j)
                if (g + j < n_groups)
                    desc[g + j] = (P << 15) | (((w[u] & 0xFFFFu) + j) << 6) | (min(64u, cnt - 64u * j) - 1u);
        }
    }
    const uint32_t sum = wave_sum_u32(mine);
    if ((threadIdx.x & 63u) == 0u) s_red[threadIdx.x >> 6] = sum;
    __syncthreads();
    if (threadIdx.x == 0) {
        const uint32_t tot = s_red[0] + s_red[1] + s_red[2] + s_red[3];
        if (tot != 0u) atomicAdd(&work[d], tot);
    }
}

__global__ __launch_bounds__(256) void k_pm_range_table(const uint32_t* __restrict__ work, uint32_t* __restrict__ range_start,
                                                        uint32_t* __restrict__ max_load) {
    __shared__ uint32_t s_red[4];
    const uint32_t lane = threadIdx.x & 63u, wv = threadIdx.x >> 6;
    const uint32_t c = work[threadIdx.x];
    const uint32_t inc = wave_incl_scan_add(c);
    const uint32_t mx = wave_max_u32(c);
    if (lane == 63u) s_red[wv] = inc;
    __syncthreads();
    uint32_t base = 0;
    for (uint32_t x = 0; x < wv; ++x) base += s_red[x];
    range_start[threadIdx.x] = base + inc - c;
    if (threadIdx.x == 255u) range_start[256] = base + inc;
    __syncthreads();
    if (lane == 0u) s_red[wv] = mx;
    __syncthreads();
    if (threadIdx.x == 0) max_load[0] = max(max(s_red[0], s_red[1]), max(s_red[2], s_red[3]));
}

__global__ __launch_bounds__(1024) void k_pm_offsets(const uint16_t* __restrict__ keys16, const uint32_t* __restrict__ desc,
                                                     const uint32_t* __restrict__ Tp, uint32_t pitch,
                                                     const uint32_t* __restrict__ range_start ,
                                                     uint32_t shift, uint32_t stride, uint32_t ltot, uint32_t* __restrict__ boff,
                                                     uint32_t* __restrict__ empty_positions) {
    extern __shared__ uint32_t s_cnt32[];
#define PADDED(i) ((i) + ((i) >> 5))
    __shared__ uint32_t s_wsum[16], s_esum[16];
    const uint32_t range = blockIdx.x, width = 1u << shift, pos0 = range << shift;
    const uint32_t lo_p = Tp[(size_t)range * pitch], hi_p = Tp[(size_t)(range + 1) * pitch];
    const uint32_t g0 = lo_p >> 6, n_ws = (hi_p - lo_p) >> 6;
    const uint32_t lo = range_start[range];
    for (uint32_t i = threadIdx.x; i < width; i += blockDim.x) s_cnt32[PADDED(i)] = 0;
    __syncthreads();
    const uint32_t lane = threadIdx.x & 63u, nw = blockDim.x >> 6;
    const uint32_t w = (uint32_t)__builtin_amdgcn_readfirstlane((int)(threadIdx.x >> 6));
    const uint32_t sub = lane >> 4, l16 = lane & 15u;
    constexpr int kU = 4;
    const uint32_t n_quads = (n_ws + 3u) >> 2;
    for (uint32_t q0 = w; q0 < n_quads; q0 += kU * nw) {
        uint2 v[kU];
        uint32_t nv[kU];
#pragma unroll
        for (int u = 0; u < kU; ++u) {
            const uint32_t q = q0 + (uint32_t)u * nw;
            uint32_t dsc = 0;
            bool has = false;
            if (q < n_quads) {
                const uint32_t ws = 4u * q;
                const uint32_t d0 = desc[g0 + ws];
                const uint32_t d1 = ws + 1 < n_ws ? desc[g0 + ws + 1] : 0u;
                const uint32_t d2 = ws + 2 < n_ws ? desc[g0 + ws + 2] : 0u;
                const uint32_t d3 = ws + 3 < n_ws ? desc[g0 + ws + 3] : 0u;
                dsc = sub == 0 ? d0 : sub == 1 ? d1 : sub == 2 ? d2 : d3;
                has = ws + sub < n_ws;
            }
            const PmSlot at = pm_unpack<true>(dsc, has, stride);
            nv[u] = at.nv;
            v[u] = *reinterpret_cast<const uint2*>(keys16 + at.slot0 + 4u * l16);
        }
#pragma unroll
        for (int u = 0; u < kU; ++u) {
            const uint32_t e = 4u * l16;
            if (e < nv[u]) atomicAdd(&s_cnt32[PADDED(v[u].x & 0xFFFFu)], 1u);
            if (e + 1 < nv[u]) atomicAdd(&s_cnt32[PADDED(v[u].x >> 16)], 1u);
            if (e + 2 < nv[u]) atomicAdd(&s_cnt32[PADDED(v[u].y & 0xFFFFu)], 1u);
            if (e + 3 < nv[u]) atomicAdd(&s_cnt32[PADDED(v[u].y >> 16)], 1u);
        }
    }
    __syncthreads();
    const uint32_t per = width >= 1024u ? width >> 10 : 1u;
    const uint32_t firstp = threadIdx.x * per;
    uint32_t sum = 0, empties = 0;
    if (firstp < width)
        for (uint32_t qq = 0; qq < per; ++qq) {
            const uint32_t cq = s_cnt32[PADDED(firstp + qq)];
            sum += cq;
            empties += (cq == 0 && pos0 + firstp + qq < ltot) ? 1u : 0u;
        }
    const uint32_t inc = wave_incl_scan_add(sum);
    const uint32_t wv = threadIdx.x >> 6;
    if (lane == 63) s_wsum[wv] = inc;
    if (empty_positions != nullptr) {
        empties = wave_sum_u32(empties);
        if (lane == 0) s_esum[wv] = empties;
    }
    __syncthreads();
    if (empty_positions != nullptr && threadIdx.x == 0) {
        uint32_t total = 0;
        for (uint32_t x = 0; x < nw; ++x) total += s_esum[x];
        if (total != 0) atomicAdd(empty_positions, total);
    }
    uint32_t run = lo + inc - sum;
    for (uint32_t x = 0; x < wv; ++x) run += s_wsum[x];
    if (firstp < width)
        for (uint32_t qq = 0; qq < per; ++qq) {
            const uint32_t cq = s_cnt32[PADDED(firstp + qq)];
            s_cnt32[PADDED(firstp + qq)] = run;
            run += cq;
        }
    __syncthreads();
    for (uint32_t i = threadIdx.x; i < width; i += blockDim.x)
        if (pos0 + i <= ltot) boff[pos0 + i] = s_cnt32[PADDED(i)];
#undef PADDED
}

struct EvQuota { const uint32_t* sev; const uint32_t* lastns; const uint64_t* poff; uint32_t n_contigs, ell; };

__global__ __launch_bounds__(1024) void k_pm_walk(const uint16_t* __restrict__ keys16, const uint16_t* __restrict__ idx16,
                                                  const uint32_t* __restrict__ desc,
                                                  const uint32_t* __restrict__ Tp, uint32_t pitch,
                                                  const uint32_t* __restrict__ range_start ,
                                                  uint32_t shift, uint32_t stride, uint32_t ltot,
                                                  const uint32_t* __restrict__ boff, const uint32_t* __restrict__ selend,
                                                  EvQuota evq,
                                                  unsigned long long* __restrict__ mask,
                                                  uint2* __restrict__ amb_lists, int lists_by_records,
                                                  uint32_t* __restrict__ amb_count ,
                                                  unsigned long long* __restrict__ kept_total) {
    extern __shared__ int32_t s_q[];
    __shared__ uint32_t s_namb, s_kept;
    __shared__ uint32_t s_ring[16][128];
    const uint32_t range = blockIdx.x, width = 1u << shift, pos0 = range << shift;
    const uint32_t live = pos0 < ltot ? min(width, ltot - pos0) : 0u;
    const uint32_t tid = threadIdx.x, nthreads = blockDim.x;
    const uint32_t lane = tid & 63u;
    const uint32_t w = (uint32_t)__builtin_amdgcn_readfirstlane((int)(tid >> 6));
    const uint32_t lo_p = Tp[(size_t)range * pitch];
    const uint32_t hi_p = Tp[(size_t)(range + 1) * pitch];
    if (tid == 0) amb_count[range] = 0;
    if (lo_p >= hi_p) return;
    const uint32_t g0 = lo_p >> 6, n_ws = (hi_p - lo_p) >> 6;
    const uint32_t n_chunks = (n_ws + 15u) >> 4;
    const uint32_t lo_true = range_start[range];
    uint2* const amb = amb_lists + (lists_by_records ? (size_t)lo_true : (size_t)range * width);
    if (evq.sev != nullptr) {
        for (uint32_t i0 = tid; i0 < live; i0 += 8 * nthreads) {
            uint32_t src[8], back[8];
#pragma unroll
            for (int u = 0; u < 8; ++u) {
                const uint32_t p = pos0 + min(i0 + u * nthreads, live - 1);
                uint32_t c_lo = 0, c_hi = evq.n_contigs;
                while (c_hi - c_lo > 1) {
                    const uint32_t mid = (c_lo + c_hi) >> 1;
                    if ((uint32_t)evq.poff[mid] <= p) c_lo = mid; else c_hi = mid;
                }
                const uint32_t base = (uint32_t)evq.poff[c_lo];
                const uint32_t k = (p - base) / evq.ell;
                src[u] = p;
                back[u] = k - evq.lastns[(size_t)(base / (4u * evq.ell) + c_lo) * 4u + k];
            }
#pragma unroll
            for (int u = 0; u < 8; ++u) src[u] = evq.sev[src[u] - back[u] * evq.ell];
#pragma unroll
            for (int u = 0; u < 8; ++u)
                if (i0 + u * nthreads < live) s_q[i0 + u * nthreads] = (int32_t)src[u];
        }
    } else
    for (uint32_t i0 = tid; i0 < live; i0 += 8 * nthreads) {
        uint32_t a[8], b[8];
#pragma unroll
        for (int u = 0; u < 8; ++u) {
            const uint32_t i = min(i0 + u * nthreads, live - 1);
            a[u] = selend[pos0 + i];
            b[u] = boff[pos0 + i];
        }
#pragma unroll
        for (int u = 0; u < 8; ++u)
            if (i0 + u * nthreads < live) s_q[i0 + u * nthreads] = (int32_t)(a[u] - b[u]);
    }
    if (tid == 0) { s_namb = 0; s_kept = 0; }
    __syncthreads();

#define QMCP_PM_RING "v96", "v97", "v98", "v99", "v100", "v101", "v102", "v103", "v104", "v105", "v106", "v107", "v108", "v109", "v110", "v111", "v112", "v113", "v114", "v115", "v116", "v117", "v118", "v119"
#define QMCP_PM_KEYREG(k) "v" QMCP_PM_STR(QMCP_PM_CAT(QMCP_PM_KEY_, k))
#define QMCP_PM_DSCREG(k) "v" QMCP_PM_STR(QMCP_PM_CAT(QMCP_PM_DSC_, k))
#define QMCP_PM_IDXREG(k) "v" QMCP_PM_STR(QMCP_PM_CAT(QMCP_PM_IDX_, k))
#define QMCP_PM_STR(x) QMCP_PM_STR2(x)
#define QMCP_PM_STR2(x) #x
#define QMCP_PM_CAT(a, b) QMCP_PM_CAT2(a, b)
#define QMCP_PM_CAT2(a, b) a##b
#define QMCP_PM_KEY_0 96
#define QMCP_PM_KEY_1 97
#define QMCP_PM_KEY_2 98
#define QMCP_PM_KEY_3 99
#define QMCP_PM_KEY_4 100
#define QMCP_PM_KEY_5 101
#define QMCP_PM_KEY_6 102
#define QMCP_PM_KEY_7 103
#define QMCP_PM_DSC_0 104
#define QMCP_PM_DSC_1 105
#define QMCP_PM_DSC_2 106
#define QMCP_PM_DSC_3 107
#define QMCP_PM_DSC_4 108
#define QMCP_PM_DSC_5 109
#define QMCP_PM_DSC_6 110
#define QMCP_PM_DSC_7 111
#define QMCP_PM_IDX_0 112
#define QMCP_PM_IDX_1 113
#define QMCP_PM_IDX_2 114
#define QMCP_PM_IDX_3 115
#define QMCP_PM_IDX_4 116
#define QMCP_PM_IDX_5 117
#define QMCP_PM_IDX_6 118
#define QMCP_PM_IDX_7 119
    static_assert(kRankDepth == 8, "the ring registers are named for eight slots");
    struct Slot { uint32_t slot0, nv, read0; bool has; };
    auto desc_offset = [&](uint32_t c) -> uint32_t {
        return (g0 + min(16u * c + w, n_ws - 1u)) * 4u;
    };
    auto slot_of = [&](uint32_t dsc, uint32_t c) -> Slot {
        const bool has = 16u * c + w < n_ws;
        const PmSlot at = pm_unpack<true>(dsc, has, stride);
        Slot s;
        s.slot0 = at.slot0;
        s.nv = at.nv;
        s.read0 = at.pass * (uint32_t)kPmPass;
        s.has = has;
        return s;
    };
    uint32_t kept = 0;
    uint32_t cur = 0, flushed = 0;
    uint32_t* const ring = s_ring[w];
#define QMCP_PM_STEP(K, KF)                                                                                                   \
    {                                                                                                                         \
        const uint32_t c = c0 + (uint32_t)(K);                                                                                \
        uint32_t key, dsc, idx;                                                                                               \
        asm volatile("s_waitcnt vmcnt(19)\n\tv_mov_b32 %0, " QMCP_PM_KEYREG(K) "\n\tv_mov_b32 %1, " QMCP_PM_DSCREG(K)          \
                     "\n\tv_mov_b32 %2, " QMCP_PM_IDXREG(K)                                                                   \
                     : "=v"(key), "=v"(dsc), "=v"(idx) : : QMCP_PM_RING, "memory");                                                      \
        const Slot at = S[K];                                                                                                 \
        const bool valid = lane < at.nv;                                                                                      \
        int32_t old = 0;                                                                                                      \
        if (valid) old = atomicSub(&s_q[key], 1);                                         \
        S[KF] = slot_of(dsc, c + 7u);                                                                                         \
        asm volatile("global_load_ushort " QMCP_PM_KEYREG(KF) ", %0, %1\n\tglobal_load_ushort " QMCP_PM_IDXREG(KF) ", %0, %2"   \
                     "\n\tglobal_load_dword " QMCP_PM_DSCREG(K) ", %3, %4"                                                    \
                     : : "v"((S[KF].slot0 + lane) * 2u), "s"(keys16), "s"(idx16), "v"(desc_offset(c + 15u)), "s"(desc)        \
                     : QMCP_PM_RING, "memory");                                                                               \
        __syncthreads();                                                                                                      \
        int32_t aft = 0;                                                                                                      \
        if (valid) aft = s_q[key];                                                                                            \
        const bool keep = valid && old > 0 && aft >= 0;                                                                       \
        if (valid && old == 1 && aft < 0) {                                                                                   \
            const uint32_t k = atomicAdd(&s_namb, 1u);                                                                        \
            amb[k] = make_uint2((c << 15) | key, (uint32_t)(-aft));                                 \
        }                                                                                                                     \
        __syncthreads();                                               \
        if (at.has) {                                                    \
            const uint64_t kb = __ballot(keep);                                                                               \
            const uint32_t cw = (uint32_t)__popcll(kb);                                                                       \
            if (keep) ring[(cur + __builtin_amdgcn_mbcnt_hi((uint32_t)(kb >> 32), __builtin_amdgcn_mbcnt_lo((uint32_t)kb, 0u))) & 127u] = at.read0 + idx; \
            cur += cw;                                                                                                        \
            if (cur - flushed >= 64u) {                                                                          \
                const uint32_t v = ring[(flushed + lane) & 127u];                                                             \
                atomicOr(&mask[v >> 6], 1ull << (v & 63u));                                                                   \
                flushed += 64u;                                                                                               \
            }                                                                                                                 \
        }                                                                                                                     \
    }
    Slot S[kRankDepth];
    {
        uint32_t d0[kRankDepth - 1];
#pragma unroll
        for (int k = 0; k < kRankDepth - 1; ++k) d0[k] = desc[desc_offset((uint32_t)k) / 4u];
#pragma unroll
        for (int k = 0; k < kRankDepth - 1; ++k) S[k] = slot_of(d0[k], (uint32_t)k);
        S[kRankDepth - 1] = Slot{0u, 0u, 0u, false};
#define QMCP_PM_ASK_KEYS(K) asm volatile("global_load_ushort " QMCP_PM_KEYREG(K) ", %0, %1\n\tglobal_load_ushort " QMCP_PM_IDXREG(K) ", %0, %2" : : "v"((S[K].slot0 + lane) * 2u), "s"(keys16), "s"(idx16) : QMCP_PM_RING, "memory");
#define QMCP_PM_ASK_DSC(K) asm volatile("global_load_dword " QMCP_PM_DSCREG(K) ", %0, %1" : : "v"(desc_offset(7u + (uint32_t)(K))), "s"(desc) : QMCP_PM_RING, "memory");
        QMCP_PM_ASK_KEYS(0) QMCP_PM_ASK_KEYS(1) QMCP_PM_ASK_KEYS(2) QMCP_PM_ASK_KEYS(3) QMCP_PM_ASK_KEYS(4) QMCP_PM_ASK_KEYS(5) QMCP_PM_ASK_KEYS(6)
        QMCP_PM_ASK_DSC(0) QMCP_PM_ASK_DSC(1) QMCP_PM_ASK_DSC(2) QMCP_PM_ASK_DSC(3) QMCP_PM_ASK_DSC(4) QMCP_PM_ASK_DSC(5) QMCP_PM_ASK_DSC(6) QMCP_PM_ASK_DSC(7)
        asm volatile("s_waitcnt vmcnt(0)" : : : QMCP_PM_RING, "memory");
#undef QMCP_PM_ASK_KEYS
#undef QMCP_PM_ASK_DSC
    }
    for (uint32_t c0 = 0; c0 < n_chunks; c0 += kRankDepth) {
        QMCP_PM_STEP(0, 7) QMCP_PM_STEP(1, 0) QMCP_PM_STEP(2, 1) QMCP_PM_STEP(3, 2)
        QMCP_PM_STEP(4, 3) QMCP_PM_STEP(5, 4) QMCP_PM_STEP(6, 5) QMCP_PM_STEP(7, 6)
    }
#undef QMCP_PM_STEP
    asm volatile("s_waitcnt vmcnt(0)" : : : QMCP_PM_RING, "memory");
    if (lane < cur - flushed) {
        const uint32_t v = ring[(flushed + lane) & 127u];
        atomicOr(&mask[v >> 6], 1ull << (v & 63u));
    }
    kept = cur;
    if (lane == 0 && kept) atomicAdd(&s_kept, kept);
    __syncthreads();
    if (tid == 0) {
        amb_count[range] = s_namb;
        if (s_kept) atomicAdd(kept_total, (unsigned long long)s_kept);
    }
}

static constexpr uint32_t kPmSettleY = 2;
static constexpr uint32_t kPmSettleWaves = 16;
__global__ __launch_bounds__(1024) void k_pm_settle(const uint16_t* __restrict__ keys16, const uint16_t* __restrict__ idx16,
                                                   const uint32_t* __restrict__ desc, const uint32_t* __restrict__ Tp,
                                                   uint32_t pitch, const uint32_t* __restrict__ range_start, uint32_t shift,
                                                   uint32_t stride, const uint2* __restrict__ amb_lists, int lists_by_records,
                                                   const uint32_t* __restrict__ amb_count,
                                                   unsigned long long* __restrict__ mask,
                                                   unsigned long long* __restrict__ kept_total) {
    __shared__ uint32_t s_kept;
    const uint32_t range = blockIdx.x, width = 1u << shift;
    const uint32_t namb = amb_count[range];
    if (blockIdx.y * kPmSettleWaves >= namb) return;
    if (threadIdx.x == 0) s_kept = 0;
    __syncthreads();
    const uint32_t lane = threadIdx.x & 63u;
    const uint32_t w = (uint32_t)__builtin_amdgcn_readfirstlane((int)(threadIdx.x >> 6));
    const uint32_t lo_p = Tp[(size_t)range * pitch], hi_p = Tp[(size_t)(range + 1) * pitch];
    const uint32_t g0 = lo_p >> 6, n_ws = (hi_p - lo_p) >> 6;
    const uint2* const amb = amb_lists + (lists_by_records ? (size_t)range_start[range] : (size_t)range * width);
    const uint64_t gt_mask = lane == 63 ? 0ull : ~((2ull << lane) - 1ull);
    uint32_t kept = 0;
    constexpr int kSteps = 16, kE = 2;
    const uint32_t stride_k = kPmSettleWaves * gridDim.y;
    for (uint32_t k0 = blockIdx.y * kPmSettleWaves + w; k0 < namb; k0 += kE * stride_k) {
        uint32_t key[kE][kSteps], dscv[kE] , p[kE], skip[kE], c_of[kE];
#pragma unroll
        for (int x = 0; x < kE; ++x) {
            const uint32_t k = k0 + (uint32_t)x * stride_k;
            const uint2 ent = k < namb ? amb[k] : make_uint2(0u, 0u);
            c_of[x] = ent.x >> 15;
            p[x] = k < namb ? ent.x & 0x7FFFu : 0xFFFFFFFFu;
            skip[x] = ent.y;
            const uint32_t ws = 16u * c_of[x] + (lane & 15u);
            dscv[x] = ws < n_ws ? desc[g0 + ws] : 0u;
        }
#pragma unroll
        for (int x = 0; x < kE; ++x) {
#pragma unroll
            for (int t = 0; t < kSteps; ++t) {
                const uint32_t dsc = (uint32_t)__builtin_amdgcn_readlane((int)dscv[x], t);
                key[x][t] = keys16[pm_unpack<false>(dsc, 16u * c_of[x] + (uint32_t)t < n_ws, stride).slot0 + lane];
            }
        }
#pragma unroll
        for (int x = 0; x < kE; ++x) {
#pragma unroll
            for (int t = kSteps - 1; t >= 0; --t) {
                const uint32_t dsc = (uint32_t)__builtin_amdgcn_readlane((int)dscv[x], t);
                const PmSlot at = pm_unpack<false>(dsc, 16u * c_of[x] + (uint32_t)t < n_ws, stride);
                const bool member = lane < at.nv && key[x][t] == p[x];
                const uint64_t m = __ballot(member);
                if (m == 0) continue;
                const uint32_t above = (uint32_t)__popcll(m & gt_mask);
                if (member && above >= skip[x]) {
                    const uint32_t v = at.pass * (uint32_t)kPmPass + idx16[at.slot0 + lane];
                    atomicOr(&mask[v >> 6], 1ull << (v & 63u));
                }
                const uint32_t in_step = (uint32_t)__popcll(m);
                kept += in_step > skip[x] ? in_step - skip[x] : 0u;
                skip[x] = skip[x] > in_step ? skip[x] - in_step : 0u;
            }
        }
    }
    if (lane == 0 && kept) atomicAdd(&s_kept, kept);
    __syncthreads();
    if (threadIdx.x == 0 && s_kept) atomicAdd(kept_total, (unsigned long long)s_kept);
}

uint32_t pm_pitch(uint32_t n) { return part_pass_pitch(n); }
uint32_t pm_pass() { return (uint32_t)kPmPass; }
uint32_t pm_stride(uint32_t ltot, uint32_t shift) { return pm_stride_of((ltot >> shift) + 1u); }
size_t pm_slots(uint32_t n, uint32_t ltot, uint32_t shift) { return (size_t)pm_pitch(n) * pm_stride(ltot, shift); }
uint32_t pm_work_words() { return kPmWorkWords; }
uint32_t pm_exc_slots(uint32_t n) { return pm_pitch(n) * kPmWaves * kPmExcPerWave + kNuOverflow; }
void launch_pm_prepare_sort(hipStream_t st, const uint32_t* starts, const uint32_t* ends, uint32_t n,
                            const uint64_t* d_roff, const uint64_t* d_poff, uint32_t n_contigs, uint32_t shift, uint32_t ltot,
                            uint16_t* keys16, uint16_t* idx16, uint32_t* cnt_tab, uint32_t* lst_tab,
                            uint32_t* work, uint32_t* stats, unsigned long long* zero_mask, uint32_t ell_reg, uint32_t* exc,
                            uint32_t exc_cap, uint32_t* exc_cnt) {
    const uint32_t pitch = pm_pitch(n);
    if (pitch == 0) return;
    (void)hipFuncSetAttribute((const void*)k_pm_prepare_sort, hipFuncAttributeMaxDynamicSharedMemorySize, (int)kPmSortLds);
    hipLaunchKernelGGL(k_pm_prepare_sort, dim3(pitch / kPmPassesPerWg), dim3(kPmThreads), kPmSortLds, st, starts, ends, n,
                       d_roff, d_poff, n_contigs, shift, pm_stride(ltot, shift), keys16, idx16, cnt_tab, lst_tab, pitch,
                       work, stats, zero_mask, exc != nullptr ? ell_reg : 0u, exc, exc_cap, exc_cnt);
    if (exc != nullptr && ell_reg != 0u)
        hipLaunchKernelGGL(k_nu_count_groups, dim3(32), dim3(256), 0, st, exc_cnt, pitch * kPmWaves, stats);
}
void launch_pm_descr(hipStream_t st, const uint32_t* Tp, const uint32_t* lstw, uint32_t n, uint32_t ltot, uint32_t shift,
                     uint32_t* desc, uint32_t* work, uint32_t* range_start, uint32_t* max_load) {
    const uint32_t pitch = pm_pitch(n), n_ranges = (ltot >> shift) + 1u;
    const uint32_t s64 = pm_stride(ltot, shift) / 64u;
    hipLaunchKernelGGL(k_pm_descr, dim3(n_ranges, kPmDescrY), dim3(256), 0, st, Tp, lstw, pitch, pitch * s64, desc, work);
    hipLaunchKernelGGL(k_pm_range_table, dim3(1), dim3(256), 0, st, work, range_start, max_load);
}
void launch_pm_offsets(hipStream_t st, const uint16_t* keys16, const uint32_t* desc, const uint32_t* Tp, uint32_t n,
                       const uint32_t* range_start, uint32_t shift, uint32_t ltot, uint32_t* boff, uint32_t* empty_positions) {
    const uint32_t n_ranges = (ltot >> shift) + 1;
    const size_t width = (size_t)1 << shift;
    const size_t lds = (width + width / 32 + 1) * sizeof(uint32_t);
    (void)hipFuncSetAttribute((const void*)k_pm_offsets, hipFuncAttributeMaxDynamicSharedMemorySize, (int)lds);
    hipLaunchKernelGGL(k_pm_offsets, dim3(n_ranges), dim3(1024), lds, st, keys16, desc, Tp, pm_pitch(n), range_start, shift,
                       pm_stride(ltot, shift), ltot, boff, empty_positions);
}
void launch_pm_walk(hipStream_t st, const uint16_t* keys16, const uint16_t* idx16, const uint32_t* desc, const uint32_t* Tp,
                    uint32_t n, const uint32_t* range_start, uint32_t shift, uint32_t ltot, const uint32_t* boff,
                    const uint32_t* selend, unsigned long long* mask, unsigned long long* kept_total, void* scratch,
                    bool scratch_by_records, uint32_t* amb_count, const uint32_t* ev_sev, const uint32_t* ev_lastns,
                    const uint64_t* d_poff, uint32_t n_contigs, uint32_t ell) {
    const uint32_t n_ranges = (ltot >> shift) + 1;
    const EvQuota evq{ev_sev, ev_lastns, d_poff, n_contigs, ell};
    const size_t lds = (((size_t)1 << shift) + 1) * sizeof(uint32_t);
    (void)hipFuncSetAttribute((const void*)k_pm_walk, hipFuncAttributeMaxDynamicSharedMemorySize, (int)lds);
    hipLaunchKernelGGL(k_pm_walk, dim3(n_ranges), dim3(1024), lds, st, keys16, idx16, desc, Tp, pm_pitch(n), range_start, shift,
                       pm_stride(ltot, shift), ltot, boff, selend, evq, mask, (uint2*)scratch, scratch_by_records ? 1 : 0,
                       amb_count, kept_total);
}
void launch_pm_settle(hipStream_t st, const uint16_t* keys16, const uint16_t* idx16, const uint32_t* desc, const uint32_t* Tp,
                      uint32_t n, const uint32_t* range_start, uint32_t shift, uint32_t ltot, const void* scratch,
                      bool scratch_by_records, const uint32_t* amb_count, unsigned long long* mask,
                      unsigned long long* kept_total) {
    const uint32_t n_ranges = (ltot >> shift) + 1;
    hipLaunchKernelGGL(k_pm_settle, dim3(n_ranges, kPmSettleY), dim3(64 * kPmSettleWaves), 0, st, keys16, idx16, desc, Tp, pm_pitch(n),
                       range_start, shift, pm_stride(ltot, shift), (const uint2*)scratch, scratch_by_records ? 1 : 0, amb_count,
                       mask, kept_total);
}
```

genome-downsampler_amd/csrc/qmcp_kernels.h:

```cpp
#ifndef QMCP_KERNELS_H
#define QMCP_KERNELS_H
#include <hip/hip_runtime.h>
#include <stdint.h>

#include "qmcp_hip.h"
#include "sweep_plan.h"
#include "dedup_plan.h"

namespace qmcp {

static constexpr uint32_t kMaxLdsRingSpan = 16383;
static constexpr uint32_t kMaxGeneralSpan = (1u << 24) - 1;
static constexpr uint32_t kMaxUniformSpan = 512;
static constexpr uint32_t kMaxCachedSpan = 4032;

void launch_prepare(hipStream_t st, const uint32_t* starts, const uint32_t* ends, uint32_t n,
                    const uint64_t* d_roff, const uint64_t* d_poff, uint32_t n_contigs,
                    const uint64_t* keep_mask, uint32_t* gstart, uint32_t* cstart,
                    uint32_t* stats, uint32_t part_shift,
                    uint32_t* part_hist ,
                    uint32_t* digit0_hist ,
                    uint32_t* global_digit_hist ,
                    unsigned long long* zero_mask ,
                    uint32_t ell_reg = 0, uint32_t* exc = nullptr, uint32_t exc_cap = 0, uint32_t* exc_cnt = nullptr
                    );
uint32_t prepare_exc_slots(uint32_t n);
void launch_general_keys(hipStream_t st, bool wide, const uint32_t* gstart, const uint32_t* starts,
                         const uint32_t* ends, uint32_t n, uint32_t span_bits, uint32_t max_span,
                         const uint64_t* keep_mask, void* keys, uint32_t* ecnt,
                         uint32_t ecnt_len );
uint32_t scan_spine_entries(uint32_t n);
void launch_exclusive_scan(hipStream_t st, const uint32_t* in, uint32_t n, uint32_t* out,
                           uint32_t* spine, bool write_total);
uint32_t sort_tiles(uint32_t n);
void launch_radix_hist(hipStream_t st, bool wide, const void* keys_in, uint32_t n, uint32_t shift,
                       uint32_t* hist);
void launch_radix_scatter(hipStream_t st, bool wide, const void* keys_in, const uint32_t* vals_in,
                          uint32_t n, uint32_t shift, const uint32_t* offs, void* keys_out,
                          uint32_t* vals_out);
uint32_t part_pass_pitch(uint32_t n);
size_t sweep_segment_words(uint32_t n_contigs, uint32_t n_windows);
const uint32_t* launch_sweep_segments(hipStream_t st, const uint32_t* boff, const uint32_t* eoff,
                                      const uint64_t* d_poff, uint32_t n_contigs, uint32_t ltot, uint32_t ell,
                                      uint32_t M, uint32_t n_windows, uint32_t* seg_words,
                                      const uint32_t* other_cov = nullptr );
bool launch_sweep_uniform_gen(hipStream_t st, const uint32_t* boff, const uint64_t* d_poff,
                              uint32_t n_contigs, uint32_t ell, uint32_t M, uint32_t ltot,
                              uint32_t* selend, uint32_t* iter_stats, const uint32_t* seg,
                              uint32_t n_seg_max, uint32_t* selend_run_in = nullptr,
                              const uint32_t* redo_in = nullptr,
                              const int32_t* nadj = nullptr ,
                              const uint32_t* own_marks = nullptr );
const uint32_t* launch_sweep_segments_speculative(hipStream_t st, const uint64_t* d_poff, uint32_t n_contigs,
                                                  uint32_t ltot, uint32_t n_windows, uint32_t burn,
                                                  uint32_t* seg_words, uint32_t* n_speculative,
                                                  uint32_t run_ins_apart, uint32_t tier);
void launch_spec_verify(hipStream_t st, const uint32_t* seg, uint32_t n_cand, uint32_t ell,
                        const uint32_t* owned, const uint32_t* run_in, uint32_t* mismatches,
                        const uint32_t* redo_in, uint32_t* redo_out,
                        const uint32_t* own_marks = nullptr );
bool launch_sweep_uniform_mw(hipStream_t st, const uint32_t* boff, const uint64_t* d_poff,
                             uint32_t n_contigs, uint32_t ell, uint32_t M, uint32_t ltot,
                             uint32_t* selend, uint32_t* iter_stats, const uint32_t* seg,
                             uint32_t n_seg_max);
size_t sweep_ev_pack_bytes(uint32_t ltot, uint32_t ell, uint32_t n_wg);
size_t sweep_ev_last_bytes(uint32_t ltot, uint32_t ell, uint32_t n_wg);
bool launch_sweep_ev_pack(hipStream_t st, const uint32_t* boff, const uint64_t* d_poff, uint32_t n_contigs,
                          uint32_t ell, uint32_t M, uint32_t ltot, const uint32_t* seg, uint32_t n_seg_max,
                          uint32_t* pk, const int32_t* nadj = nullptr, const uint32_t* from = nullptr);
bool launch_sweep_ev_chain(hipStream_t st, const uint32_t* boff, const uint64_t* d_poff, uint32_t n_contigs,
                           uint32_t ell, uint32_t M, uint32_t ltot, const uint32_t* seg, uint32_t n_seg_max,
                           const uint32_t* pk, uint32_t* sev, uint32_t* lastns, uint32_t* iter_stats,
                           const int32_t* nadj = nullptr, uint32_t* ckpt = nullptr ,
                           const uint32_t* restart = nullptr );
size_t sweep_ev_ckpt_bytes(uint32_t ltot, uint32_t ell, uint32_t n_wg);
bool launch_sweep_ev_expand(hipStream_t st, const uint32_t* boff, const uint64_t* d_poff, uint32_t n_contigs,
                            uint32_t ell, uint32_t M, uint32_t ltot, const uint32_t* seg, uint32_t n_seg_max,
                            const uint32_t* sev, const uint32_t* lastns, uint32_t* selend, const uint32_t* from = nullptr);
bool launch_sweep_uniform(hipStream_t st, const uint32_t* boff, const uint64_t* d_poff,
                          uint32_t n_contigs, uint32_t ell, uint32_t M, uint32_t ltot,
                          uint32_t* selend, uint32_t* iter_stats, const uint32_t* seg,
                          uint32_t n_seg_max);
void launch_sweep_general(hipStream_t st, bool wide, const uint32_t* boff, const uint32_t* eoff,
                          const void* skeys, const uint64_t* d_poff, uint32_t n_contigs,
                          uint32_t span_bits, uint32_t max_span, uint32_t M, uint32_t* selend,
                          uint32_t ring_size, const uint32_t* seg, uint32_t n_seg_max,
                          uint32_t* g_rings );
void launch_group_heads(hipStream_t st, bool wide, const void* sorted, uint32_t n,
                        uint32_t* next_head );
void launch_sweep_general_cached(hipStream_t st, bool wide, const uint32_t* boff,
                                 const uint32_t* eoff, const void* sorted, const uint32_t* next_head,
                                 const uint64_t* d_poff, uint32_t n_contigs, uint32_t span_bits,
                                 uint32_t max_span, uint32_t M, uint32_t* selend, uint32_t ring,
                                 const uint32_t* seg, uint32_t n_seg_max);
bool launch_sweep_general_reg(hipStream_t st, bool wide, const uint32_t* boff, const uint32_t* eoff,
                              const void* sorted, const uint32_t* next_head, const uint64_t* d_poff,
                              uint32_t n_contigs, uint32_t span_bits, uint32_t max_span, uint32_t M,
                              uint32_t* selend, const uint32_t* seg, uint32_t n_seg_max,
                              uint32_t* selend_odd = nullptr, const uint32_t* redo_in = nullptr,
                              uint32_t* snap = nullptr );
size_t spec_snap_bytes(uint32_t n_cand);
void launch_spec_verify_merge_mixed(hipStream_t st, const uint32_t* seg, uint32_t n_cand, uint32_t max_span,
                                    uint32_t* out_even, const uint32_t* out_odd, const uint32_t* snap,
                                    uint32_t* mismatches, const uint32_t* redo_in, uint32_t* redo_out);
void launch_mark(hipStream_t st, bool wide, const void* sorted, const uint32_t* svals, uint32_t ltot,
                 const uint32_t* boff, const uint32_t* selend, uint64_t* mask,
                 unsigned long long* n_kept);
void launch_profile_need(hipStream_t st, const uint32_t* boff, const uint32_t* eoff, uint32_t ltot, const uint32_t* rs,
                         const uint32_t* re, const uint32_t* cap, uint32_t n_regions, uint32_t default_cap, uint32_t* need,
                         unsigned long long* pstat);
const uint32_t* launch_profile_segments(hipStream_t st, const uint32_t* need, const uint64_t* d_poff, uint32_t n_contigs,
                                        uint32_t ltot, uint32_t n_windows, uint32_t* seg_words);
bool launch_sweep_general_reg_capped(hipStream_t st, bool wide, const uint32_t* boff, const uint32_t* need,
                                     const void* sorted, const uint32_t* next_head, const uint64_t* d_poff,
                                     uint32_t n_contigs, uint32_t span_bits, uint32_t max_span, uint32_t* selend,
                                     const uint32_t* seg, uint32_t n_seg_max);
void launch_sweep_general_capped(hipStream_t st, bool wide, const uint32_t* boff, const uint32_t* need, const void* sorted,
                                 const uint64_t* d_poff, uint32_t n_contigs, uint32_t span_bits, uint32_t max_span,
                                 uint32_t* selend, uint32_t ring_size, const uint32_t* seg, uint32_t n_seg_max,
                                 uint32_t* g_rings);
void launch_bucket_heads(hipStream_t st, bool wide, const void* sorted, const uint32_t* svals,
                         uint32_t n, uint32_t span_bits, uint32_t ltot, uint32_t* boff);
void launch_reverse_min_scan(hipStream_t st, uint32_t* data, uint32_t n, uint32_t* spine);
void launch_radix_hist_rec(hipStream_t st, bool first, const uint32_t* keys, const void* recs,
                           uint32_t n, uint32_t shift, uint32_t* hist);
void launch_radix_scatter_rec(hipStream_t st, bool first, const uint32_t* keys, const void* recs_in,
                              uint32_t n, uint32_t shift, const uint32_t* offs, void* recs_out);
void launch_coverage(hipStream_t st, const uint32_t* boff, const uint32_t* eoff, uint32_t ltot,
                     uint32_t* cov);
void launch_b_and_demand(hipStream_t st, const uint32_t* cov, uint32_t n, uint32_t M, int32_t* b, int32_t* d);
void launch_complete_pairs(hipStream_t st, uint64_t* mask, uint32_t n_words, uint64_t n_reads);
void launch_word_popcounts(hipStream_t st, const uint64_t* words, uint32_t n_words, uint32_t* counts);
void launch_mask_to_indices(hipStream_t st, const uint64_t* mask, uint32_t n_words, const uint32_t* word_base,
                            unsigned long long* out);
void launch_compact_pairs(hipStream_t st, const uint32_t* starts, const uint32_t* ends,
                          const uint64_t* pair_keep, const uint32_t* word_base, uint64_t n_pairs,
                          uint32_t* starts_c, uint32_t* ends_c, uint32_t* orig_pair);
void launch_expand_mask(hipStream_t st, const uint64_t* mask_c, const uint32_t* orig_pair,
                        uint32_t n_reads_c, uint64_t* mask);
void launch_amplicon_filter(hipStream_t st, const uint32_t* starts, const uint32_t* ends,
                            const uint32_t* seq_lengths, const uint32_t* qualities,
                            uint64_t n_pairs, const uint32_t* amp_starts, const uint32_t* amp_ends,
                            uint32_t n_amp, uint32_t min_length, uint32_t min_mapq,
                            uint64_t* pair_keep);

uint32_t range_shift_for(uint32_t ltot);
bool range_path_supported(uint32_t ltot);
bool range_path_two_level(uint32_t ltot);
uint32_t seg_tile_bound(uint32_t n);
void launch_partition_level1(hipStream_t st, const uint32_t* starts, const uint64_t* d_roff,
                             const uint64_t* d_poff, uint32_t n_contigs, uint32_t n, uint32_t shift_hi,
                             const uint32_t* offs, void* recs_out, uint32_t* super_start,
                             uint32_t* max_super_load, const uint32_t* ends = nullptr, uint32_t ell_reg = 0);
void launch_partition_level2(hipStream_t st, const void* recs_in, uint32_t n, uint32_t shift,
                             uint32_t* tables , uint32_t* hist, uint32_t* spine,
                             uint16_t* keys16_out, uint32_t* idx_out, uint32_t* range_start ,
                             uint32_t* max_load);
void launch_range_partition(hipStream_t st, const uint32_t* gstart_or_null, const uint32_t* starts,
                            const uint64_t* d_roff, const uint64_t* d_poff, uint32_t n_contigs,
                            uint32_t n, uint32_t shift, const uint32_t* offs, uint16_t* keys16_out,
                            uint32_t* idx_out, uint32_t* range_start , uint32_t* max_load,
                            const uint32_t* ends = nullptr, uint32_t ell_reg = 0 );
void launch_gstart(hipStream_t st, const uint32_t* starts, uint32_t n, const uint64_t* d_roff,
                   const uint64_t* d_poff, uint32_t n_contigs, uint32_t* gstart);
void launch_fill_ends(hipStream_t st, const uint32_t* starts, uint32_t n, uint32_t span_minus_1, uint32_t* ends);
void launch_range_offsets(hipStream_t st, const uint16_t* keys16, const uint32_t* range_start,
                          uint32_t shift, uint32_t ltot, uint32_t* boff,
                          uint32_t* empty_positions );
size_t rank_scratch_bytes(uint32_t shift, uint32_t ltot, uint32_t n);
bool rank_scratch_by_records(uint32_t shift, uint32_t ltot, uint32_t n);
void launch_rank_mark(hipStream_t st, const uint16_t* keys16, const uint32_t* idx,
                      const uint32_t* range_start, uint32_t shift, uint32_t ltot, const uint32_t* boff,
                      const uint32_t* selend, unsigned long long* mask, unsigned long long* kept_total,
                      void* scratch, bool scratch_by_records);

uint32_t pm_pitch(uint32_t n);
uint32_t pm_pass();
uint32_t pm_stride(uint32_t ltot, uint32_t shift);
size_t pm_slots(uint32_t n, uint32_t ltot, uint32_t shift);
uint32_t pm_work_words();
void launch_pm_prepare_sort(hipStream_t st, const uint32_t* starts, const uint32_t* ends, uint32_t n,
                            const uint64_t* d_roff, const uint64_t* d_poff, uint32_t n_contigs, uint32_t shift, uint32_t ltot,
                            uint16_t* keys16, uint16_t* idx16, uint32_t* cnt_tab, uint32_t* lst_tab,
                            uint32_t* work ,
                            uint32_t* stats, unsigned long long* zero_mask, uint32_t ell_reg = 0, uint32_t* exc = nullptr,
                            uint32_t exc_cap = 0, uint32_t* exc_cnt = nullptr);
uint32_t pm_exc_slots(uint32_t n);
void launch_pm_descr(hipStream_t st, const uint32_t* Tp, const uint32_t* lstw, uint32_t n, uint32_t ltot, uint32_t shift,
                     uint32_t* desc, uint32_t* work, uint32_t* range_start, uint32_t* max_load);
void launch_pm_offsets(hipStream_t st, const uint16_t* keys16, const uint32_t* desc, const uint32_t* Tp, uint32_t n,
                       const uint32_t* range_start, uint32_t shift, uint32_t ltot, uint32_t* boff, uint32_t* empty_positions);
void launch_pm_walk(hipStream_t st, const uint16_t* keys16, const uint16_t* idx16, const uint32_t* desc, const uint32_t* Tp,
                    uint32_t n, const uint32_t* range_start, uint32_t shift, uint32_t ltot, const uint32_t* boff,
                    const uint32_t* selend, unsigned long long* mask, unsigned long long* kept_total, void* scratch,
                    bool scratch_by_records, uint32_t* amb_count,
                    const uint32_t* ev_sev = nullptr, const uint32_t* ev_lastns = nullptr,
                    const uint64_t* d_poff = nullptr, uint32_t n_contigs = 0, uint32_t ell = 0);
void launch_pm_settle(hipStream_t st, const uint16_t* keys16, const uint16_t* idx16, const uint32_t* desc, const uint32_t* Tp,
                      uint32_t n, const uint32_t* range_start, uint32_t shift, uint32_t ltot, const void* scratch,
                      bool scratch_by_records, const uint32_t* amb_count, unsigned long long* mask,
                      unsigned long long* kept_total);


void launch_span_mode_share(hipStream_t st, const uint32_t* starts, const uint32_t* ends, uint32_t n, uint32_t* out );
size_t nu_exc_bytes(uint32_t cap);
uint32_t* nu_exc_counts(uint32_t* exc, uint32_t cap);
void launch_nu_count_span(hipStream_t st, const uint32_t* starts, const uint32_t* ends, uint32_t n, uint32_t span, uint32_t* out);
void launch_nu_setup(hipStream_t st, uint32_t* exc, uint32_t cap, uint32_t n_exc, const uint32_t* n_over ,
                     const uint32_t* boff, uint32_t ltot, uint32_t ell, uint32_t M, uint32_t* ce ,
                     uint32_t* spine, int32_t* nadj , uint32_t* state );
void launch_nu_round(hipStream_t st, uint32_t* exc, uint32_t cap, uint32_t n_exc, const uint32_t* n_over, bool first_round,
                     const uint32_t* boff, const uint32_t* selend, int32_t* nadj, const uint32_t* ce ,
                     const uint64_t* d_poff, uint32_t n_contigs,
                     uint32_t ell, uint32_t M, uint2* suspects, uint32_t suspects_cap, uint32_t* state,
                     unsigned long long* viol_key, uint32_t* viol_idx,
                     const uint32_t* swept_from ,
                     uint32_t* sweep_from_next ,
                     uint32_t ltot, uint32_t* spine ,
                     const uint32_t* seg_exact , uint32_t n_cand,
                     uint32_t* marks_next ,
                     uint32_t* selend_prev ,
                     uint32_t* dirty ,
                     uint32_t* dirty_next,
                     const uint32_t* seg_fine = nullptr ,
                     uint32_t* fine_next = nullptr );
size_t nu_cells_bytes();
size_t nu_suspect_bytes(uint32_t suspects_cap);
void launch_nu_mark_selected(hipStream_t st, uint32_t* exc, uint32_t cap, uint32_t n_exc, const uint32_t* n_over,
                             unsigned long long* mask, unsigned long long* kept_total);

void launch_bc_keys(hipStream_t st, const uint32_t* starts, const uint32_t* ends, const uint32_t* ids, uint32_t n,
                    const uint32_t* lengths, uint32_t n_contigs, uint32_t* keys, uint32_t* err);
void launch_bc_bounds(hipStream_t st, const void* sorted, uint32_t n, uint32_t n_groups, uint32_t* offs);
void launch_bc_gather(hipStream_t st, const void* sorted, uint32_t n, const uint32_t* starts, const uint32_t* ends,
                      uint32_t* starts_out, uint32_t* ends_out);
void launch_bc_scatter_mask(hipStream_t st, const uint64_t* batch_mask, const void* sorted, uint32_t n, uint64_t* mask);

void launch_ladder_compact(hipStream_t st, bool first, const uint32_t* starts, const uint32_t* ends,
                           const void* origin_in, const uint64_t* mask, const uint32_t* word_base, uint32_t n,
                           uint32_t* starts_c, uint32_t* ends_c, uint32_t* origin_c);
void launch_ladder_offsets(hipStream_t st, const uint32_t* offs, uint32_t n_contigs, const uint64_t* mask,
                           const uint32_t* word_base, uint32_t* next);
void launch_ladder_levels(hipStream_t st, bool first, const uint64_t* mask, const void* origin_in, uint32_t n,
                          uint32_t level, uint8_t* levels);

static constexpr uint32_t kStratumTallyTile = 1024;
void launch_st_keys(hipStream_t st, const uint32_t* starts, const uint32_t* ends, const uint32_t* ids,
                    const uint32_t* strata, uint32_t n, const uint32_t* lengths, uint32_t n_contigs, uint32_t n_strata,
                    uint32_t* keys, uint32_t* err);
void launch_st_tally(hipStream_t st, const void* sorted, uint32_t n_placed, uint32_t n_contigs, const uint32_t* starts,
                     const uint32_t* ends, const uint64_t* mask, uint64_t* rows);

void launch_amplicon_filter_by_contig(hipStream_t st, const uint32_t* starts, const uint32_t* ends, const uint32_t* ids,
                                      const uint32_t* seq_lengths, const uint32_t* qualities, uint64_t n_pairs,
                                      const uint32_t* lengths, uint32_t n_contigs, const uint32_t* amp_offs,
                                      const uint32_t* amp_starts, const uint32_t* amp_pmax, uint32_t n_amp,
                                      uint32_t min_length, uint32_t min_mapq, uint64_t* pair_keep, uint32_t* err);
void launch_compact_pairs_ids(hipStream_t st, const uint32_t* starts, const uint32_t* ends, const uint32_t* ids,
                              const uint64_t* pair_keep, const uint32_t* word_base, uint64_t n_pairs, uint32_t* starts_c,
                              uint32_t* ends_c, uint32_t* ids_c, uint32_t* orig_pair);

void launch_qc_range(hipStream_t st, const uint32_t* q, const uint32_t* ids, uint32_t n, uint32_t* range);
void launch_qc_keys(hipStream_t st, bool wide, const uint32_t* starts, const uint32_t* ends, const uint32_t* q,
                    const uint32_t* ids, const uint64_t* roff, const uint64_t* poff, uint32_t n_contigs, uint64_t ltot,
                    uint32_t n, uint32_t min_span, uint32_t span_bits, uint32_t q_max, uint32_t q_bits, void* keys);
void launch_qc_marks(hipStream_t st, bool wide, const void* sorted, const uint32_t* svals, uint32_t n, uint32_t q_bits,
                     const uint64_t* mask, uint32_t* kb, uint32_t* seg_end, uint32_t* seg_head_rev);
void launch_qc_choose(hipStream_t st, bool wide, const void* sorted, const uint32_t* svals, uint32_t n,
                      const uint32_t* P, const uint32_t* seg_end, const uint32_t* seg_head_rev, uint64_t* mask,
                      unsigned long long* counters);

void launch_target_project(hipStream_t st, const uint32_t* starts, const uint32_t* ends, const uint32_t* ids, uint32_t n,
                           const uint32_t* lengths, uint32_t n_contigs, const uint32_t* offs, const uint32_t* rs,
                           const uint32_t* re, const uint32_t* cum, uint32_t n_regions, uint32_t* ps, uint32_t* pe,
                           uint64_t* on, uint64_t* off, uint32_t* err);
void launch_compact_reads(hipStream_t st, const uint32_t* ps, const uint32_t* pe, const uint32_t* ids, const uint32_t* q,
                          const uint32_t* remap, const uint64_t* on, const uint32_t* word_base, uint32_t n,
                          uint32_t* starts_c, uint32_t* ends_c, uint32_t* ids_c, uint32_t* q_c, uint32_t* orig);
void launch_expand_mask_reads(hipStream_t st, const uint64_t* mask_c, const uint32_t* orig, uint32_t n_c, uint64_t* mask);
void launch_or_words(hipStream_t st, uint64_t* mask, const uint64_t* other, uint32_t n_words);

void launch_depth_events(hipStream_t st, const uint32_t* starts, const uint32_t* ends, const uint32_t* ids, uint32_t n,
                         const uint64_t* mask, const uint32_t* lengths, const uint32_t* boff, uint32_t n_contigs,
                         uint32_t c0, uint32_t c1, uint64_t* ev, uint64_t* counts, uint32_t* err);
uint32_t depth_lds_contigs();
uint32_t depth_chunks(uint32_t positions);
void launch_depth_sums(hipStream_t st, const uint64_t* ev, uint32_t positions, uint64_t* sums);
void launch_depth_consume(hipStream_t st, const uint64_t* ev, uint32_t positions, const uint64_t* sums, uint32_t M,
                          const uint32_t* c_lo, const uint32_t* c_hi, const uint32_t* c_row, uint32_t n_c,
                          const uint32_t* r_lo, const uint32_t* r_hi, const uint32_t* r_row, uint32_t n_r,
                          bool scope_regions, uint32_t n_rows, uint64_t* acc64, uint32_t* acc32, uint32_t n_bins,
                          uint64_t* hist);

void launch_track_count(hipStream_t st, const uint64_t* ev, uint32_t positions, const uint64_t* sums, uint32_t M,
                        uint32_t flags, uint32_t depth_cap, const uint32_t* s_lo, const uint32_t* s_hi, uint32_t n_s,
                        uint32_t* cnt, uint64_t* totals);
void launch_track_emit(hipStream_t st, const uint64_t* ev, uint32_t positions, const uint64_t* sums, uint32_t M,
                       uint32_t flags, uint32_t depth_cap, const uint32_t* s_lo, const uint32_t* s_hi, uint32_t n_s,
                       const uint32_t* c_lo, const uint32_t* c_hi, const uint32_t* c_row, uint32_t n_c,
                       const uint32_t* cnt, qmcp_hip_track_run* runs);

uint32_t dedup_hist_max();
void launch_dd_range(hipStream_t st, const uint32_t* starts, const uint32_t* ends, const uint32_t* ids,
                     const uint32_t* tags, const uint32_t* q, uint32_t n, const uint32_t* lengths, uint32_t n_contigs,
                     bool pairs, uint32_t* out);
void launch_dd_read_keys(hipStream_t st, uint32_t key_bytes, const uint32_t* starts, const uint32_t* ends,
                         const uint32_t* ids, const uint32_t* tags, const uint32_t* q, const uint32_t* idx,
                         const uint64_t* poff, uint64_t ltot, uint32_t n, uint32_t min_span, uint32_t tag_min,
                         uint32_t q_max, const DedupPack& pack, void* keys);
void launch_dd_pair_keys(hipStream_t st, uint32_t key_bytes, const uint32_t* cid, const uint32_t* q, const uint32_t* idx,
                         uint32_t n_units, uint32_t idu, uint32_t q_min, uint32_t score_max, const DedupPack& pack,
                         void* keys);
void launch_dd_heads(hipStream_t st, uint32_t form, const void* sorted, const uint32_t* svals, uint32_t low_bits,
                     uint32_t n_act, const uint32_t* starts, const uint32_t* ends, const uint32_t* ids,
                     const uint32_t* tags, const uint32_t* cid, uint32_t* flag);
void launch_dd_cell_ids(hipStream_t st, const uint32_t* vals, uint32_t stride, const uint32_t* E, uint32_t n_placed,
                        uint32_t n, uint32_t idu, uint32_t* cid);
void launch_dd_segments(hipStream_t st, bool pairs, const uint32_t* vals, uint32_t stride, const uint32_t* E,
                        uint32_t n_act, uint64_t* surv, uint64_t* dup, uint32_t* headpos);
void launch_dd_family_stats(hipStream_t st, const uint32_t* headpos, const uint32_t* n_fam, uint32_t n_act,
                            uint32_t hist_bins, uint64_t* hist, uint64_t* counters);
void launch_dd_compact(hipStream_t st, const uint32_t* starts, const uint32_t* ends, const uint32_t* ids,
                       const uint64_t* surv, const uint32_t* word_base, uint32_t n, uint32_t* starts_c, uint32_t* ends_c,
                       uint32_t* ids_c, uint32_t* orig);

uint32_t pair_credit_pad();
void launch_pair_gather_mask(hipStream_t st, const void* sorted, uint32_t n, const uint64_t* mask, uint64_t* in_bits,
                             uint64_t* rest_bits);
void launch_pair_credit_events(hipStream_t st, const void* sorted, uint32_t n, const uint64_t* in_bits,
                               const uint32_t* starts, const uint32_t* ends, const uint32_t* pos_off, uint32_t first_contig,
                               uint32_t* ev);
void launch_pair_need(hipStream_t st, const uint32_t* boff, const uint32_t* eoff, const uint32_t* credit, uint32_t ltot,
                      uint32_t target, uint32_t* need, unsigned long long* pstat);
void launch_pair_count_bits(hipStream_t st, const uint64_t* mask, uint32_t n_words, unsigned long long* count);

}
#endif
```

profiles/summarize_pmc.py:

```python
#!/usr/bin/env python3
import collections
import csv
import json
import os
import re
import sys

CALIB_BYTES = 512 << 20
KERNEL_WIDTHS = {
    "k_prepare": ("read_4", "write_16"),
    "k_range_partition": ("read_4", "write_4"),
    "k_range_offsets": ("read_8", "write_4"),
    "k_rank_mark": ("rw_2_4", "atomic_or64"),
    "k_pm_prepare_sort": ("read_4", "write_4"),
    "k_pm_offsets": ("read_8", "write_4"),
    "k_pm_rank_mark": ("read_2", "atomic_or64"),
    "k_pm_descr": ("read_4", "write_4"),
    "k_pm_range_table": ("read_4", "write_4"),
    "k_pm_walk": ("read_2", "atomic_or64"),
    "k_pm_settle": ("read_2", "atomic_or64"),
    "k_sweep_pack": ("read_4", "write_16"),
    "k_sweep_uniform_ev": ("read_16", "write_4"),
    "k_sweep_expand": ("read_4", "write_4"),
}


def short(name):
    m = re.search(r"(k_\w+|calib_\w+<[^>]*>|calib_\w+)", name)
    return m.group(1) if m else name[:40]


def load(path, counter):
    acc = collections.defaultdict(list)
    with open(path) as f:
        for row in csv.DictReader(f):
            if row["Counter_Name"] == counter:
                acc[short(row["Kernel_Name"])].append(float(row["Counter_Value"]))
    return acc


def calib_key(kernel):
    if kernel.startswith("calib_rw_2_4"):
        return "rw_2_4"
    if kernel.startswith("calib_atomic_or64"):
        return "atomic_or64"
    m = re.match(r"calib_(read|write)<(.*)>", kernel)
    if not m:
        return None
    width = {"unsigned short": 2, "unsigned int": 4}.get(m.group(2))
    if width is None:
        width = 8 if "2" in m.group(2) else 16
    return f"{m.group(1)}_{width}"


def calibrate(src, out):
    fetch = load(os.path.join(src, "calib_FETCH_SIZE", "pmc_counter_collection.csv"), "FETCH_SIZE")
    write = load(os.path.join(src, "calib_WRITE_SIZE", "pmc_counter_collection.csv"), "WRITE_SIZE")
    res = {"fetch": {}, "write": {}, "raw_kb": {}}
    for k in sorted(set(fetch) | set(write)):
        key = calib_key(k)
        if key is None:
            continue
        f = sum(fetch.get(k, [0])) / max(len(fetch.get(k, [])), 1)
        w = sum(write.get(k, [0])) / max(len(write.get(k, [])), 1)
        res["raw_kb"][key] = {"fetch_kb": round(f, 1), "write_kb": round(w, 1)}
        moved = CALIB_BYTES // 6 * 6 if key == "rw_2_4" else CALIB_BYTES
        if key.startswith("read") or key == "rw_2_4":
            res["fetch"][key] = round(moved / (f * 1024), 4) if f else None
        if key.startswith("write"):
            res["write"][key] = round(moved / (w * 1024), 4) if w else None
        if key == "atomic_or64":
            res["atomic_or64"] = {"fetch_bytes_per_atomic": round(f * 1024 / (4 << 20), 2),
                                  "write_bytes_per_atomic": round(w * 1024 / (4 << 20), 2)}
    res["_note"] = ("bytes moved per KiB the counter reports, by access width (lab/pmc_calib.hip: 512 MiB per kernel, "
                    "coalesced); 1.0 = the counter is exact, 2.0 = it reports half")
    json.dump(res, open(out, "w"), indent=1)
    print(json.dumps(res, indent=1))


def summarize(src, prefix, out, calib_path, note):
    fetch = load(os.path.join(src, prefix + "pmc_FETCH_SIZE", "pmc_counter_collection.csv"), "FETCH_SIZE")
    write = load(os.path.join(src, prefix + "pmc_WRITE_SIZE", "pmc_counter_collection.csv"), "WRITE_SIZE")
    calib = json.load(open(calib_path)) if calib_path and os.path.exists(calib_path) else {"fetch": {}, "write": {}}
    res = {}
    for k in sorted(set(fetch) | set(write)):
        f = sum(fetch.get(k, [0])) / max(len(fetch.get(k, [])), 1)
        w = sum(write.get(k, [0])) / max(len(write.get(k, [])), 1)
        rkey, wkey = KERNEL_WIDTHS.get(k, ("read_4", "write_4"))
        ff = calib["fetch"].get(rkey) or 2.0
        wf = (calib["write"].get(wkey) or 1.0) if wkey != "atomic_or64" else 1.0
        res[k] = {"launches": len(fetch.get(k, write.get(k, []))), "fetch_kb": round(f, 1), "write_kb": round(w, 1),
                  "fetch_factor": ff, "write_factor": wf, "hbm_bytes_per_launch": int((ff * f + wf * w) * 1024)}
    per_solve = sum(v["hbm_bytes_per_launch"] for k, v in res.items() if k.startswith("k_"))
    res["_total"] = {"hbm_bytes_per_solve": per_solve}
    res["_source"] = note or "rocprofv3 --pmc FETCH_SIZE / WRITE_SIZE, one pass per counter (profiles/collect.sh)"
    res["_calibration"] = {"fetch": calib.get("fetch"), "write": calib.get("write"), "atomic_or64": calib.get("atomic_or64")}
    json.dump(res, open(out, "w"), indent=1)
    for k, v in res.items():
        if not k.startswith("_"):
            print(f"{k:28s} {v['hbm_bytes_per_launch'] / 1e6:10.1f} MB/launch  (fetch x{v['fetch_factor']}, write x{v['write_factor']})")
    print(f"{'solver kernels, per solve':28s} {per_solve / 1e6:10.1f} MB")


if __name__ == "__main__":
    if sys.argv[1] == "calibrate":
        calibrate(sys.argv[2], sys.argv[3])
    else:
        summarize(sys.argv[2], sys.argv[3], sys.argv[4], sys.argv[5] if len(sys.argv) > 5 else None,
                  sys.argv[6] if len(sys.argv) > 6 else None)
```

Baseline: 117,900.

## Fuse pass-major scan, descriptor and range-table kernels; drop settle pass

Replaces the three-kernel exclusive scan plus k_pm_descr and k_pm_range_table with two kernels. k_pm_row_sums computes per-row partial sums, and k_pm_tables performs the scan in place while also building descriptors, range starts and max load. The scalars clear is folded into the tables kernel, and the per-solve stats init now copies from pinned host memory. The separate k_pm_settle launch and the work-buffer zeroing are removed, which cuts launch count and passes over the histogram, but only works if the walk kernel now handles the ambiguous cases that settle used to resolve.

Measured after the change: 121,600 (median of 6 runs). +3.1%, better.

```diff
diff --git a/genome-downsampler_amd/csrc/api/context.inc.hip b/genome-downsampler_amd/csrc/api/context.inc.hip
--- a/genome-downsampler_amd/csrc/api/context.inc.hip
+++ b/genome-downsampler_amd/csrc/api/context.inc.hip
@@ -115,6 +115,7 @@
     uint32_t last_iters = 0, last_blocks = 0;
     SolveRun run;
     uint32_t* h_head = nullptr;
+    uint32_t* h_stats_init = nullptr;
     hipEvent_t ev_head = nullptr;
     hipEvent_t ev_done = nullptr;
     bool mixed_seen = false;
diff --git a/genome-downsampler_amd/csrc/api/near_uniform_route.inc.hip b/genome-downsampler_amd/csrc/api/near_uniform_route.inc.hip
--- a/genome-downsampler_amd/csrc/api/near_uniform_route.inc.hip
+++ b/genome-downsampler_amd/csrc/api/near_uniform_route.inc.hip
@@ -42,7 +42,7 @@
             return QMCP_OK;
         }
         c->nu_ell = ell;
-        if (run.pm) TRY(queue_pm_head(c, st, ell));
+        if (run.pm) TRY(queue_pm_head(c, st, ell, true));
         else TRY(queue_rm_head(c, st, ell, true));
         uint32_t* d_max_load = (uint32_t*)c->ranges.p + 65540;
         HIP_TRY(hipMemcpyAsync(c->h_nu, d_max_load, sizeof(uint32_t), hipMemcpyDeviceToHost, st));
diff --git a/genome-downsampler_amd/csrc/api/solve_head.inc.hip b/genome-downsampler_amd/csrc/api/solve_head.inc.hip
--- a/genome-downsampler_amd/csrc/api/solve_head.inc.hip
+++ b/genome-downsampler_amd/csrc/api/solve_head.inc.hip
@@ -1,5 +1,5 @@
 int queue_rm_head(qmcp_hip_ctx* c, hipStream_t s1, uint32_t filter, bool clear_mask);
-int queue_pm_head(qmcp_hip_ctx* c, hipStream_t st, uint32_t filter);
+int queue_pm_head(qmcp_hip_ctx* c, hipStream_t st, uint32_t filter, bool rerun);
 
 bool pm_route_ok(const qmcp_hip_ctx* c, const uint64_t* roff, const Problem& pr, uint32_t shift) {
     if (c->opt.pass_major < 0) return false;
@@ -59,7 +59,7 @@
         if (may_pm) {
             const size_t groups = pm_bytes / (64 * sizeof(uint16_t));
             TRY(ensure(c, c->pm_desc, groups * sizeof(uint32_t)));
-            TRY(ensure(c, c->pm_work, 1024 * sizeof(uint32_t)));
+            TRY(ensure(c, c->pm_work, (size_t)qmcp::pm_work_words() * sizeof(uint32_t)));
         }
         TRY(ensure(c, c->vals[0], (size_t)n * sizeof(uint32_t)));
         TRY(ensure(c, c->vals[1], (size_t)n * sizeof(uint32_t)));
@@ -110,13 +110,12 @@
     } else {
         run.have_gstart = false;
         hipStream_t s1 = c->stream;
-        static const uint32_t init[8] = {0xFFFFFFFFu, 0u, 0u, 0u, 0u, 0u, 0u, 0u};
-        HIP_TRY(hipMemcpyAsync(c->stats.p, init, sizeof(init), hipMemcpyHostToDevice, s1));
+        HIP_TRY(hipMemcpyAsync(c->stats.p, c->h_stats_init, 8 * sizeof(uint32_t), hipMemcpyHostToDevice, s1));
         run.pm = !two_level && pm_route_ok(c, roff, pr, range_shift);
         run.nu_filter = c->nu_ell;
         hs[5] = hs[6] = 0;
         if (run.pm) {
-            TRY(queue_pm_head(c, s1, run.nu_filter));
+            TRY(queue_pm_head(c, s1, run.nu_filter, false));
         } else {
             TRY(queue_rm_head(c, s1, run.nu_filter, true));
         }
@@ -198,34 +197,32 @@
     return QMCP_OK;
 }
 
-int queue_pm_head(qmcp_hip_ctx* c, hipStream_t st, uint32_t filter) {
+int queue_pm_head(qmcp_hip_ctx* c, hipStream_t st, uint32_t filter, bool rerun) {
     SolveRun& run = c->run;
     const uint32_t n = (uint32_t)run.pr.n, ltot = (uint32_t)run.pr.ltot, n_contigs = run.n_contigs;
     uint32_t* d_stats = (uint32_t*)c->stats.p;
-    static const uint32_t zeros[4] = {0u, 0u, 0u, 0u};
-    HIP_TRY(hipMemcpyAsync(d_stats + 3, zeros, sizeof(zeros), hipMemcpyHostToDevice, st));
+    if (rerun) HIP_TRY(hipMemcpyAsync(d_stats + 3, c->h_stats_init + 1, 4 * sizeof(uint32_t), hipMemcpyHostToDevice, st));
     uint32_t* d_range_start = (uint32_t*)c->ranges.p;
     uint32_t* d_max_load = d_range_start + 65540;
     {
         KernelSpan sp(c, "k_pm_prepare_sort", st);
         qmcp::launch_pm_prepare_sort(st, run.d_starts, run.d_ends, n, (const uint64_t*)c->roff.p, (const uint64_t*)c->poff.p,
                                      n_contigs, run.range_shift, ltot, (uint16_t*)c->keys[0].p, (uint16_t*)c->keys[1].p,
-                                     (uint32_t*)c->hist2.p, (uint32_t*)c->hist.p,
-                                     (uint32_t*)c->pm_work.p, d_stats, (unsigned long long*)run.d_mask, filter,
+                                     (uint32_t*)c->hist2.p, (uint32_t*)c->hist.p, d_stats, (unsigned long long*)run.d_mask, filter,
                                      filter ? (uint32_t*)c->nu_exc.p : nullptr, nu_cap_for(n),
                                      filter ? qmcp::nu_exc_counts((uint32_t*)c->nu_exc.p, nu_cap_for(n)) : nullptr);
     }
     HIP_TRY(hipGetLastError());
     HIP_TRY(hipEventRecord(c->ev[EV_PREP], st));
     {
-        KernelSpan sp(c, "scan_radix_hist(3 kernels)", st);
-        qmcp::launch_exclusive_scan(st, (const uint32_t*)c->hist2.p, 256u * qmcp::pm_pitch(n), (uint32_t*)c->hist2.p,
-                                    (uint32_t*)c->spine2.p, true);
-    }
-    {
-        KernelSpan sp(c, "k_pm_descr + k_pm_range_table", st);
-        qmcp::launch_pm_descr(st, (const uint32_t*)c->hist2.p, (const uint32_t*)c->hist.p, n, ltot, run.range_shift,
-                              (uint32_t*)c->pm_desc.p, (uint32_t*)c->pm_work.p, d_range_start, d_max_load);
+        KernelSpan sp(c, "k_pm_row_sums", st);
+        qmcp::launch_pm_row_sums(st, (const uint32_t*)c->hist2.p, (const uint32_t*)c->hist.p, n, (uint32_t*)c->pm_work.p);
+    }
+    {
+        KernelSpan sp(c, "k_pm_tables", st);
+        qmcp::launch_pm_tables(st, (uint32_t*)c->hist2.p, (const uint32_t*)c->hist.p, n, ltot, run.range_shift,
+                               (uint32_t*)c->pm_desc.p, (const uint32_t*)c->pm_work.p, d_range_start, d_max_load,
+                               rerun ? nullptr : (uint32_t*)c->scalars.p);
     }
     HIP_TRY(hipEventRecord(c->ev_fork, st));
     {
@@ -242,20 +239,10 @@
     SolveRun& run = c->run;
     const uint32_t n = (uint32_t)run.pr.n, ltot = (uint32_t)run.pr.ltot;
     const bool by_records = qmcp::rank_scratch_by_records(run.range_shift, ltot, n);
-    const uint16_t* keys16 = (const uint16_t*)c->keys[0].p;
-    const uint16_t* idx16 = (const uint16_t*)c->keys[1].p;
-    const uint32_t* desc = (const uint32_t*)c->pm_desc.p;
-    const uint32_t* Tp = (const uint32_t*)c->hist2.p;
-    const uint32_t* range_start = (const uint32_t*)c->ranges.p;
-    uint32_t* amb_count = (uint32_t*)c->pm_work.p + 512;
-    unsigned long long* kept_total = (unsigned long long*)c->scalars.p;
-    {
-        KernelSpan sp(c, "k_pm_walk", st);
-        qmcp::launch_pm_walk(st, keys16, idx16, desc, Tp, n, range_start, run.range_shift, ltot, (const uint32_t*)c->boff.p,
-                             (const uint32_t*)c->selend.p, (unsigned long long*)run.d_mask, kept_total, c->rankamb.p, by_records,
-                             amb_count, ev_sev, ev_lastns, (const uint64_t*)c->poff.p, run.n_contigs, ell);
-    }
-    KernelSpan sp(c, "k_pm_settle", st);
-    qmcp::launch_pm_settle(st, keys16, idx16, desc, Tp, n, range_start, run.range_shift, ltot, c->rankamb.p, by_records,
-                           amb_count, (unsigned long long*)run.d_mask, kept_total);
-}
+    KernelSpan sp(c, "k_pm_walk", st);
+    qmcp::launch_pm_walk(st, (const uint16_t*)c->keys[0].p, (const uint16_t*)c->keys[1].p, (const uint32_t*)c->pm_desc.p,
+                         (const uint32_t*)c->hist2.p, n, (const uint32_t*)c->ranges.p, run.range_shift, ltot,
+                         (const uint32_t*)c->boff.p, (const uint32_t*)c->selend.p, (unsigned long long*)run.d_mask,
+                         (unsigned long long*)c->scalars.p, c->rankamb.p, by_records, ev_sev, ev_lastns,
+                         (const uint64_t*)c->poff.p, run.n_contigs, ell);
+}
diff --git a/genome-downsampler_amd/csrc/api/solve_tail.inc.hip b/genome-downsampler_amd/csrc/api/solve_tail.inc.hip
--- a/genome-downsampler_amd/csrc/api/solve_tail.inc.hip
+++ b/genome-downsampler_amd/csrc/api/solve_tail.inc.hip
@@ -64,7 +64,7 @@
     uint32_t max_load_now = max_load;
     if (uniform && run.nu_filter != 0 && run.nu_filter != max_span) {
         c->nu_ell = 0;
-        if (run.pm) TRY(queue_pm_head(c, c->stream, 0));
+        if (run.pm) TRY(queue_pm_head(c, c->stream, 0, true));
         else TRY(queue_rm_head(c, c->stream, 0, true));
         HIP_TRY(hipMemcpyAsync(c->h_nu, (uint32_t*)c->ranges.p + 65540, sizeof(uint32_t), hipMemcpyDeviceToHost, c->stream));
         HIP_TRY(hipStreamSynchronize(c->stream));
@@ -99,7 +99,7 @@
     }
     if (!near_done) HIP_TRY(hipEventRecord(c->ev[EV_SCAN], c->stream));
     bool mixed_whole_contigs = false;
-    if (!near_done) HIP_TRY(hipMemsetAsync(c->scalars.p, 0, 64, c->stream));
+    if (!near_done && !(uniform && run.pm)) HIP_TRY(hipMemsetAsync(c->scalars.p, 0, 64, c->stream));
     if (uniform && may_rank) {
         hipStream_t s1 = c->stream;
         HIP_TRY(hipGetLastError());
@@ -393,7 +393,12 @@
     if (e == hipSuccess) e = hipEventCreateWithFlags(&c->ev_fork, hipEventDisableTiming);
     if (e == hipSuccess) e = hipEventCreateWithFlags(&c->ev_head, hipEventDisableTiming);
     if (e == hipSuccess) e = hipEventCreateWithFlags(&c->ev_done, hipEventDisableTiming);
-    if (e == hipSuccess) e = hipHostMalloc((void**)&c->h_head, 8 * sizeof(uint32_t), hipHostMallocDefault);
+    if (e == hipSuccess) e = hipHostMalloc((void**)&c->h_head, 16 * sizeof(uint32_t), hipHostMallocDefault);
+    if (e == hipSuccess) {
+        c->h_stats_init = c->h_head + 8;
+        c->h_stats_init[0] = 0xFFFFFFFFu;
+        for (int i = 1; i < 8; ++i) c->h_stats_init[i] = 0u;
+    }
     if (e != hipSuccess) {
         qmcp_hip_destroy(c);
         return fail(QMCP_EHIP, "context setup: %s", hipGetErrorString(e));
diff --git a/genome-downsampler_amd/csrc/kernels/pass_major.inc.hip b/genome-downsampler_amd/csrc/kernels/pass_major.inc.hip
--- a/genome-downsampler_amd/csrc/kernels/pass_major.inc.hip
+++ b/genome-downsampler_amd/csrc/kernels/pass_major.inc.hip
@@ -15,7 +15,6 @@
     uint32_t shift, uint32_t stride ,
     uint16_t* __restrict__ keys16, uint16_t* __restrict__ idx16,
     uint32_t* __restrict__ cnt_tab, uint32_t* __restrict__ lst_tab, uint32_t pitch ,
-    uint32_t* __restrict__ work ,
     uint32_t* __restrict__ stats, unsigned long long* __restrict__ zero_mask,
     uint32_t ell_reg, uint32_t* __restrict__ exc, uint32_t exc_cap, uint32_t* __restrict__ exc_cnt) {
     extern __shared__ uint32_t s_pm[];
@@ -27,7 +26,6 @@
     uint32_t* s_tabc = s_wave + 16;
     uint32_t* s_tabl = s_tabc + kPmPassesPerWg * 256;
     uint32_t* s_exc = s_tabl + kPmPassesPerWg * 256;
-    if (blockIdx.x == 0 && threadIdx.x < 260) work[threadIdx.x] = 0;
     const int lane = threadIdx.x & 63, w = threadIdx.x >> 6;
     uint32_t mn = 0xFFFFFFFFu, mx = 0, bad = 0;
     auto contig_of = [&](uint32_t i) {
@@ -253,8 +251,8 @@
     }
 }
 
-static constexpr uint32_t kPmWorkWords = 260;
 static constexpr uint32_t kPmDescrY = 8;
+static constexpr uint32_t kPmWorkWords = 256u * kPmDescrY * 2u;
 
 struct PmSlot { uint32_t slot0, nv, pass; };
 template <bool kVector>
@@ -266,61 +264,129 @@
     return s;
 }
 
-__global__ __launch_bounds__(256) void k_pm_descr(const uint32_t* __restrict__ Tp, const uint32_t* __restrict__ lstw,
-                                                  uint32_t pitch, uint32_t n_groups ,
-                                                  uint32_t* __restrict__ desc, uint32_t* __restrict__ work) {
-    __shared__ uint32_t s_red[4];
+__device__ __forceinline__ void pm_row_part(uint32_t pitch, uint32_t& P_beg, uint32_t& P_end) {
+    const uint32_t per = (pitch + kPmDescrY - 1u) / kPmDescrY;
+    P_beg = min(pitch, blockIdx.y * per);
+    P_end = min(pitch, (blockIdx.y + 1u) * per);
+}
+
+__global__ __launch_bounds__(256) void k_pm_row_sums(const uint32_t* __restrict__ cnt_tab, const uint32_t* __restrict__ lstw,
+                                                     uint32_t pitch, uint32_t* __restrict__ work) {
+    __shared__ uint32_t s_red[2][4];
     const uint32_t d = blockIdx.x;
-    const uint32_t per = (pitch + gridDim.y - 1u) / gridDim.y;
-    const uint32_t P_end = min(pitch, (blockIdx.y + 1u) * per);
-    uint32_t mine = 0;
-    for (uint32_t P0 = blockIdx.y * per + threadIdx.x; P0 < P_end; P0 += 4u * 256u) {
-        uint32_t w[4], t[4];
+    uint32_t P_beg, P_end;
+    pm_row_part(pitch, P_beg, P_end);
+    uint32_t pad = 0, tru = 0;
+    for (uint32_t P0 = P_beg + threadIdx.x; P0 < P_end; P0 += 4u * 256u) {
+        uint32_t c[4], w[4];
 #pragma unroll
         for (int u = 0; u < 4; ++u) {
             const uint32_t P = min(P0 + (uint32_t)u * 256u, P_end - 1u);
+            c[u] = cnt_tab[(size_t)d * pitch + P];
             w[u] = lstw[(size_t)d * pitch + P];
-            t[u] = Tp[(size_t)d * pitch + P];
-        }
+        }
+#pragma unroll
+        for (int u = 0; u < 4; ++u)
+            if (P0 + (uint32_t)u * 256u < P_end) { pad += c[u]; tru += w[u] >> 16; }
+    }
+    pad = wave_sum_u32(pad);
+    tru = wave_sum_u32(tru);
+    if ((threadIdx.x & 63u) == 0u) { s_red[0][threadIdx.x >> 6] = pad; s_red[1][threadIdx.x >> 6] = tru; }
+    __syncthreads();
+    if (threadIdx.x == 0) {
+        uint32_t* const out = work + ((size_t)d * kPmDescrY + blockIdx.y) * 2u;
+        out[0] = s_red[0][0] + s_red[0][1] + s_red[0][2] + s_red[0][3];
+        out[1] = s_red[1][0] + s_red[1][1] + s_red[1][2] + s_red[1][3];
+    }
+}
+
+__global__ __launch_bounds__(256) void k_pm_tables(uint32_t* tab, const uint32_t* __restrict__ lstw, uint32_t pitch,
+                                                   uint32_t n_groups ,
+                                                   uint32_t* __restrict__ desc, const uint32_t* __restrict__ work,
+                                                   uint32_t* __restrict__ range_start, uint32_t* __restrict__ max_load,
+                                                   uint32_t* __restrict__ clear16 ) {
+    __shared__ uint32_t s_red[4], s_base, s_tile[2][4][4];
+    const uint32_t d = blockIdx.x, y = blockIdx.y, tid = threadIdx.x;
+    const uint32_t lane = tid & 63u, wv = tid >> 6;
+    const bool first = d == 0u && y == 0u;
+    uint32_t rp = 0, rt = 0, before = 0;
+    {
+        const uint4* const src = reinterpret_cast<const uint4*>(work + (size_t)tid * kPmDescrY * 2u);
+        uint4 q[kPmDescrY / 2u];
+#pragma unroll
+        for (uint32_t k = 0; k < kPmDescrY / 2u; ++k) q[k] = src[k];
+#pragma unroll
+        for (uint32_t k = 0; k < kPmDescrY / 2u; ++k) {
+            if (2u * k < y) before += q[k].x;
+            if (2u * k + 1u < y) before += q[k].z;
+            rp += q[k].x + q[k].z;
+            rt += q[k].y + q[k].w;
+        }
+    }
+    {
+        const uint32_t inc = wave_incl_scan_add(rp);
+        if (lane == 63u) s_red[wv] = inc;
+        __syncthreads();
+        uint32_t base = 0;
+        for (uint32_t x = 0; x < wv; ++x) base += s_red[x];
+        if (tid == d) s_base = base + inc - rp + before;
+        if (first && tid == 255u) tab[(size_t)256u * pitch] = base + inc;
+        __syncthreads();
+    }
+    if (first) {
+        if (clear16 != nullptr && tid < 16u) clear16[tid] = 0u;
+        const uint32_t inc = wave_incl_scan_add(rt);
+        const uint32_t mx = wave_max_u32(rt);
+        if (lane == 63u) s_red[wv] = inc;
+        __syncthreads();
+        uint32_t base = 0;
+        for (uint32_t x = 0; x < wv; ++x) base += s_red[x];
+        range_start[tid] = base + inc - rt;
+        if (tid == 255u) range_start[256] = base + inc;
+        __syncthreads();
+        if (lane == 0u) s_red[wv] = mx;
+        __syncthreads();
+        if (tid == 0) max_load[0] = max(max(s_red[0], s_red[1]), max(s_red[2], s_red[3]));
+    }
+    uint32_t P_beg, P_end;
+    pm_row_part(pitch, P_beg, P_end);
+    uint32_t carry = s_base;
+    uint32_t round = 0;
+    for (uint32_t P0 = P_beg; P0 < P_end; P0 += 4u * 256u, round ^= 1u) {
+        uint32_t c[4], w[4], inc[4];
 #pragma unroll
         for (int u = 0; u < 4; ++u) {
-            const uint32_t P = P0 + (uint32_t)u * 256u;
-            const uint32_t cnt = P < P_end ? w[u] >> 16 : 0u;
+            const uint32_t P = P0 + (uint32_t)u * 256u + tid;
+            const bool in = P < P_end;
+            const size_t at = (size_t)d * pitch + min(P, P_end - 1u);
+            c[u] = tab[at];
+            w[u] = lstw[at];
+            if (!in) { c[u] = 0u; w[u] = 0u; }
+        }
+#pragma unroll
+        for (int u = 0; u < 4; ++u) {
+            inc[u] = wave_incl_scan_add(c[u]);
+            if (lane == 63u) s_tile[round][u][wv] = inc[u];
+        }
+        __syncthreads();
+#pragma unroll
+        for (int u = 0; u < 4; ++u) {
+            uint32_t base = carry;
+            for (uint32_t x = 0; x < wv; ++x) base += s_tile[round][u][x];
+            carry += s_tile[round][u][0] + s_tile[round][u][1] + s_tile[round][u][2] + s_tile[round][u][3];
+            const uint32_t P = P0 + (uint32_t)u * 256u + tid;
+            if (P >= P_end) continue;
+            const uint32_t t = base + inc[u] - c[u];
+            tab[(size_t)d * pitch + P] = t;
+            const uint32_t cnt = w[u] >> 16;
             if (cnt == 0u) continue;
-            mine += cnt;
-            const uint32_t g = t[u] >> 6;
+            const uint32_t g = t >> 6;
             const uint32_t n_ws = (cnt + 63u) >> 6;
             for (uint32_t j = 0; j < n_ws; ++j)
                 if (g + j < n_groups)
                     desc[g + j] = (P << 15) | (((w[u] & 0xFFFFu) + j) << 6) | (min(64u, cnt - 64u * j) - 1u);
         }
     }
-    const uint32_t sum = wave_sum_u32(mine);
-    if ((threadIdx.x & 63u) == 0u) s_red[threadIdx.x >> 6] = sum;
-    __syncthreads();
-    if (threadIdx.x == 0) {
-        const uint32_t tot = s_red[0] + s_red[1] + s_red[2] + s_red[3];
-        if (tot != 0u) atomicAdd(&work[d], tot);
-    }
-}
-
-__global__ __launch_bounds__(256) void k_pm_range_table(const uint32_t* __restrict__ work, uint32_t* __restrict__ range_start,
-                                                        uint32_t* __restrict__ max_load) {
-    __shared__ uint32_t s_red[4];
-    const uint32_t lane = threadIdx.x & 63u, wv = threadIdx.x >> 6;
-    const uint32_t c = work[threadIdx.x];
-    const uint32_t inc = wave_incl_scan_add(c);
-    const uint32_t mx = wave_max_u32(c);
-    if (lane == 63u) s_red[wv] = inc;
-    __syncthreads();
-    uint32_t base = 0;
-    for (uint32_t x = 0; x < wv; ++x) base += s_red[x];
-    range_start[threadIdx.x] = base + inc - c;
-    if (threadIdx.x == 255u) range_start[256] = base + inc;
-    __syncthreads();
-    if (lane == 0u) s_red[wv] = mx;
-    __syncthreads();
-    if (threadIdx.x == 0) max_load[0] = max(max(s_red[0], s_red[1]), max(s_red[2], s_red[3]));
 }
 
 __global__ __launch_bounds__(1024) void k_pm_offsets(const uint16_t* __restrict__ keys16, const uint32_t* __restrict__ desc,
@@ -411,6 +477,57 @@
 
 struct EvQuota { const uint32_t* sev; const uint32_t* lastns; const uint64_t* poff; uint32_t n_contigs, ell; };
 
+__device__ __forceinline__ uint32_t pm_settle_groups(const uint16_t* __restrict__ keys16, const uint16_t* __restrict__ idx16,
+                                                     const uint32_t* __restrict__ desc, uint32_t g0, uint32_t n_ws,
+                                                     uint32_t stride, const uint2* amb, uint32_t namb, uint32_t w,
+                                                     uint32_t lane, unsigned long long* __restrict__ mask) {
+    const uint64_t gt_mask = lane == 63 ? 0ull : ~((2ull << lane) - 1ull);
+    uint32_t kept = 0;
+    constexpr int kSteps = 16, kE = 2;
+    constexpr uint32_t stride_k = 16;
+    for (uint32_t k0 = w; k0 < namb; k0 += kE * stride_k) {
+        uint32_t key[kE][kSteps], dscv[kE] , p[kE], skip[kE], c_of[kE];
+#pragma unroll
+        for (int x = 0; x < kE; ++x) {
+            const uint32_t k = k0 + (uint32_t)x * stride_k;
+            const uint2 ent = k < namb ? amb[k] : make_uint2(0u, 0u);
+            c_of[x] = ent.x >> 15;
+            p[x] = k < namb ? ent.x & 0x7FFFu : 0xFFFFFFFFu;
+            skip[x] = ent.y;
+            const uint32_t ws = 16u * c_of[x] + (lane & 15u);
+            dscv[x] = ws < n_ws ? desc[g0 + ws] : 0u;
+        }
+#pragma unroll
+        for (int x = 0; x < kE; ++x) {
+#pragma unroll
+            for (int t = 0; t < kSteps; ++t) {
+                const uint32_t dsc = (uint32_t)__builtin_amdgcn_readlane((int)dscv[x], t);
+                key[x][t] = keys16[pm_unpack<false>(dsc, 16u * c_of[x] + (uint32_t)t < n_ws, stride).slot0 + lane];
+            }
+        }
+#pragma unroll
+        for (int x = 0; x < kE; ++x) {
+#pragma unroll
+            for (int t = kSteps - 1; t >= 0; --t) {
+                const uint32_t dsc = (uint32_t)__builtin_amdgcn_readlane((int)dscv[x], t);
+                const PmSlot at = pm_unpack<false>(dsc, 16u * c_of[x] + (uint32_t)t < n_ws, stride);
+                const bool member = lane < at.nv && key[x][t] == p[x];
+                const uint64_t m = __ballot(member);
+                if (m == 0) continue;
+                const uint32_t above = (uint32_t)__popcll(m & gt_mask);
+                if (member && above >= skip[x]) {
+                    const uint32_t v = at.pass * (uint32_t)kPmPass + idx16[at.slot0 + lane];
+                    atomicOr(&mask[v >> 6], 1ull << (v & 63u));
+                }
+                const uint32_t in_step = (uint32_t)__popcll(m);
+                kept += in_step > skip[x] ? in_step - skip[x] : 0u;
+                skip[x] = skip[x] > in_step ? skip[x] - in_step : 0u;
+            }
+        }
+    }
+    return kept;
+}
+
 __global__ __launch_bounds__(1024) void k_pm_walk(const uint16_t* __restrict__ keys16, const uint16_t* __restrict__ idx16,
                                                   const uint32_t* __restrict__ desc,
                                                   const uint32_t* __restrict__ Tp, uint32_t pitch,
@@ -420,7 +537,6 @@
                                                   EvQuota evq,
                                                   unsigned long long* __restrict__ mask,
                                                   uint2* __restrict__ amb_lists, int lists_by_records,
-                                                  uint32_t* __restrict__ amb_count ,
                                                   unsigned long long* __restrict__ kept_total) {
     extern __shared__ int32_t s_q[];
     __shared__ uint32_t s_namb, s_kept;
@@ -432,7 +548,6 @@
     const uint32_t w = (uint32_t)__builtin_amdgcn_readfirstlane((int)(tid >> 6));
     const uint32_t lo_p = Tp[(size_t)range * pitch];
     const uint32_t hi_p = Tp[(size_t)(range + 1) * pitch];
-    if (tid == 0) amb_count[range] = 0;
     if (lo_p >= hi_p) return;
     const uint32_t g0 = lo_p >> 6, n_ws = (hi_p - lo_p) >> 6;
     const uint32_t n_chunks = (n_ws + 15u) >> 4;
@@ -590,81 +705,11 @@
         atomicOr(&mask[v >> 6], 1ull << (v & 63u));
     }
     kept = cur;
+    __syncthreads();
+    kept += pm_settle_groups(keys16, idx16, desc, g0, n_ws, stride, amb, s_namb, w, lane, mask);
     if (lane == 0 && kept) atomicAdd(&s_kept, kept);
     __syncthreads();
-    if (tid == 0) {
-        amb_count[range] = s_namb;
-        if (s_kept) atomicAdd(kept_total, (unsigned long long)s_kept);
-    }
-}
-
-static constexpr uint32_t kPmSettleY = 2;
-static constexpr uint32_t kPmSettleWaves = 16;
-__global__ __launch_bounds__(1024) void k_pm_settle(const uint16_t* __restrict__ keys16, const uint16_t* __restrict__ idx16,
-                                                   const uint32_t* __restrict__ desc, const uint32_t* __restrict__ Tp,
-                                                   uint32_t pitch, const uint32_t* __restrict__ range_start, uint32_t shift,
-                                                   uint32_t stride, const uint2* __restrict__ amb_lists, int lists_by_records,
-                                                   const uint32_t* __restrict__ amb_count,
-                                                   unsigned long long* __restrict__ mask,
-                                                   unsigned long long* __restrict__ kept_total) {
-    __shared__ uint32_t s_kept;
-    const uint32_t range = blockIdx.x, width = 1u << shift;
-    const uint32_t namb = amb_count[range];
-    if (blockIdx.y * kPmSettleWaves >= namb) return;
-    if (threadIdx.x == 0) s_kept = 0;
-    __syncthreads();
-    const uint32_t lane = threadIdx.x & 63u;
-    const uint32_t w = (uint32_t)__builtin_amdgcn_readfirstlane((int)(threadIdx.x >> 6));
-    const uint32_t lo_p = Tp[(size_t)range * pitch], hi_p = Tp[(size_t)(range + 1) * pitch];
-    const uint32_t g0 = lo_p >> 6, n_ws = (hi_p - lo_p) >> 6;
-    const uint2* const amb = amb_lists + (lists_by_records ? (size_t)range_start[range] : (size_t)range * width);
-    const uint64_t gt_mask = lane == 63 ? 0ull : ~((2ull << lane) - 1ull);
-    uint32_t kept = 0;
-    constexpr int kSteps = 16, kE = 2;
-    const uint32_t stride_k = kPmSettleWaves * gridDim.y;
-    for (uint32_t k0 = blockIdx.y * kPmSettleWaves + w; k0 < namb; k0 += kE * stride_k) {
-        uint32_t key[kE][kSteps], dscv[kE] , p[kE], skip[kE], c_of[kE];
-#pragma unroll
-        for (int x = 0; x < kE; ++x) {
-            const uint32_t k = k0 + (uint32_t)x * stride_k;
-            const uint2 ent = k < namb ? amb[k] : make_uint2(0u, 0u);
-            c_of[x] = ent.x >> 15;
-            p[x] = k < namb ? ent.x & 0x7FFFu : 0xFFFFFFFFu;
-            skip[x] = ent.y;
-            const uint32_t ws = 16u * c_of[x] + (lane & 15u);
-            dscv[x] = ws < n_ws ? desc[g0 + ws] : 0u;
-        }
-#pragma unroll
-        for (int x = 0; x < kE; ++x) {
-#pragma unroll
-            for (int t = 0; t < kSteps; ++t) {
-                const uint32_t dsc = (uint32_t)__builtin_amdgcn_readlane((int)dscv[x], t);
-                key[x][t] = keys16[pm_unpack<false>(dsc, 16u * c_of[x] + (uint32_t)t < n_ws, stride).slot0 + lane];
-            }
-        }
-#pragma unroll
-        for (int x = 0; x < kE; ++x) {
-#pragma unroll
-            for (int t = kSteps - 1; t >= 0; --t) {
-                const uint32_t dsc = (uint32_t)__builtin_amdgcn_readlane((int)dscv[x], t);
-                const PmSlot at = pm_unpack<false>(dsc, 16u * c_of[x] + (uint32_t)t < n_ws, stride);
-                const bool member = lane < at.nv && key[x][t] == p[x];
-                const uint64_t m = __ballot(member);
-                if (m == 0) continue;
-                const uint32_t above = (uint32_t)__popcll(m & gt_mask);
-                if (member && above >= skip[x]) {
-                    const uint32_t v = at.pass * (uint32_t)kPmPass + idx16[at.slot0 + lane];
-                    atomicOr(&mask[v >> 6], 1ull << (v & 63u));
-                }
-                const uint32_t in_step = (uint32_t)__popcll(m);
-                kept += in_step > skip[x] ? in_step - skip[x] : 0u;
-                skip[x] = skip[x] > in_step ? skip[x] - in_step : 0u;
-            }
-        }
-    }
-    if (lane == 0 && kept) atomicAdd(&s_kept, kept);
-    __syncthreads();
-    if (threadIdx.x == 0 && s_kept) atomicAdd(kept_total, (unsigned long long)s_kept);
+    if (tid == 0 && s_kept) atomicAdd(kept_total, (unsigned long long)s_kept);
 }
 
 uint32_t pm_pitch(uint32_t n) { return part_pass_pitch(n); }
@@ -676,23 +721,29 @@
 void launch_pm_prepare_sort(hipStream_t st, const uint32_t* starts, const uint32_t* ends, uint32_t n,
                             const uint64_t* d_roff, const uint64_t* d_poff, uint32_t n_contigs, uint32_t shift, uint32_t ltot,
                             uint16_t* keys16, uint16_t* idx16, uint32_t* cnt_tab, uint32_t* lst_tab,
-                            uint32_t* work, uint32_t* stats, unsigned long long* zero_mask, uint32_t ell_reg, uint32_t* exc,
+                            uint32_t* stats, unsigned long long* zero_mask, uint32_t ell_reg, uint32_t* exc,
                             uint32_t exc_cap, uint32_t* exc_cnt) {
     const uint32_t pitch = pm_pitch(n);
     if (pitch == 0) return;
     (void)hipFuncSetAttribute((const void*)k_pm_prepare_sort, hipFuncAttributeMaxDynamicSharedMemorySize, (int)kPmSortLds);
     hipLaunchKernelGGL(k_pm_prepare_sort, dim3(pitch / kPmPassesPerWg), dim3(kPmThreads), kPmSortLds, st, starts, ends, n,
                        d_roff, d_poff, n_contigs, shift, pm_stride(ltot, shift), keys16, idx16, cnt_tab, lst_tab, pitch,
-                       work, stats, zero_mask, exc != nullptr ? ell_reg : 0u, exc, exc_cap, exc_cnt);
+                       stats, zero_mask, exc != nullptr ? ell_reg : 0u, exc, exc_cap, exc_cnt);
     if (exc != nullptr && ell_reg != 0u)
         hipLaunchKernelGGL(k_nu_count_groups, dim3(32), dim3(256), 0, st, exc_cnt, pitch * kPmWaves, stats);
 }
-void launch_pm_descr(hipStream_t st, const uint32_t* Tp, const uint32_t* lstw, uint32_t n, uint32_t ltot, uint32_t shift,
-                     uint32_t* desc, uint32_t* work, uint32_t* range_start, uint32_t* max_load) {
-    const uint32_t pitch = pm_pitch(n), n_ranges = (ltot >> shift) + 1u;
+void launch_pm_row_sums(hipStream_t st, const uint32_t* cnt_tab, const uint32_t* lstw, uint32_t n, uint32_t* work) {
+    const uint32_t pitch = pm_pitch(n);
+    if (pitch == 0) return;
+    hipLaunchKernelGGL(k_pm_row_sums, dim3(256, kPmDescrY), dim3(256), 0, st, cnt_tab, lstw, pitch, work);
+}
+void launch_pm_tables(hipStream_t st, uint32_t* tab, const uint32_t* lstw, uint32_t n, uint32_t ltot, uint32_t shift,
+                      uint32_t* desc, const uint32_t* work, uint32_t* range_start, uint32_t* max_load, uint32_t* clear16) {
+    const uint32_t pitch = pm_pitch(n);
+    if (pitch == 0) return;
     const uint32_t s64 = pm_stride(ltot, shift) / 64u;
-    hipLaunchKernelGGL(k_pm_descr, dim3(n_ranges, kPmDescrY), dim3(256), 0, st, Tp, lstw, pitch, pitch * s64, desc, work);
-    hipLaunchKernelGGL(k_pm_range_table, dim3(1), dim3(256), 0, st, work, range_start, max_load);
+    hipLaunchKernelGGL(k_pm_tables, dim3(256, kPmDescrY), dim3(256), 0, st, tab, lstw, pitch, pitch * s64, desc, work,
+                       range_start, max_load, clear16);
 }
 void launch_pm_offsets(hipStream_t st, const uint16_t* keys16, const uint32_t* desc, const uint32_t* Tp, uint32_t n,
                        const uint32_t* range_start, uint32_t shift, uint32_t ltot, uint32_t* boff, uint32_t* empty_positions) {
@@ -706,7 +757,7 @@
 void launch_pm_walk(hipStream_t st, const uint16_t* keys16, const uint16_t* idx16, const uint32_t* desc, const uint32_t* Tp,
                     uint32_t n, const uint32_t* range_start, uint32_t shift, uint32_t ltot, const uint32_t* boff,
                     const uint32_t* selend, unsigned long long* mask, unsigned long long* kept_total, void* scratch,
-                    bool scratch_by_records, uint32_t* amb_count, const uint32_t* ev_sev, const uint32_t* ev_lastns,
+                    bool scratch_by_records, const uint32_t* ev_sev, const uint32_t* ev_lastns,
                     const uint64_t* d_poff, uint32_t n_contigs, uint32_t ell) {
     const uint32_t n_ranges = (ltot >> shift) + 1;
     const EvQuota evq{ev_sev, ev_lastns, d_poff, n_contigs, ell};
@@ -714,14 +765,5 @@
     (void)hipFuncSetAttribute((const void*)k_pm_walk, hipFuncAttributeMaxDynamicSharedMemorySize, (int)lds);
     hipLaunchKernelGGL(k_pm_walk, dim3(n_ranges), dim3(1024), lds, st, keys16, idx16, desc, Tp, pm_pitch(n), range_start, shift,
                        pm_stride(ltot, shift), ltot, boff, selend, evq, mask, (uint2*)scratch, scratch_by_records ? 1 : 0,
-                       amb_count, kept_total);
-}
-void launch_pm_settle(hipStream_t st, const uint16_t* keys16, const uint16_t* idx16, const uint32_t* desc, const uint32_t* Tp,
-                      uint32_t n, const uint32_t* range_start, uint32_t shift, uint32_t ltot, const void* scratch,
-                      bool scratch_by_records, const uint32_t* amb_count, unsigned long long* mask,
-                      unsigned long long* kept_total) {
-    const uint32_t n_ranges = (ltot >> shift) + 1;
-    hipLaunchKernelGGL(k_pm_settle, dim3(n_ranges, kPmSettleY), dim3(64 * kPmSettleWaves), 0, st, keys16, idx16, desc, Tp, pm_pitch(n),
-                       range_start, shift, pm_stride(ltot, shift), (const uint2*)scratch, scratch_by_records ? 1 : 0, amb_count,
-                       mask, kept_total);
-}
+                       kept_total);
+}
diff --git a/genome-downsampler_amd/csrc/qmcp_kernels.h b/genome-downsampler_amd/csrc/qmcp_kernels.h
--- a/genome-downsampler_amd/csrc/qmcp_kernels.h
+++ b/genome-downsampler_amd/csrc/qmcp_kernels.h
@@ -182,24 +182,20 @@
 void launch_pm_prepare_sort(hipStream_t st, const uint32_t* starts, const uint32_t* ends, uint32_t n,
                             const uint64_t* d_roff, const uint64_t* d_poff, uint32_t n_contigs, uint32_t shift, uint32_t ltot,
                             uint16_t* keys16, uint16_t* idx16, uint32_t* cnt_tab, uint32_t* lst_tab,
-                            uint32_t* work ,
                             uint32_t* stats, unsigned long long* zero_mask, uint32_t ell_reg = 0, uint32_t* exc = nullptr,
                             uint32_t exc_cap = 0, uint32_t* exc_cnt = nullptr);
 uint32_t pm_exc_slots(uint32_t n);
-void launch_pm_descr(hipStream_t st, const uint32_t* Tp, const uint32_t* lstw, uint32_t n, uint32_t ltot, uint32_t shift,
-                     uint32_t* desc, uint32_t* work, uint32_t* range_start, uint32_t* max_load);
+void launch_pm_row_sums(hipStream_t st, const uint32_t* cnt_tab, const uint32_t* lstw, uint32_t n, uint32_t* work);
+void launch_pm_tables(hipStream_t st, uint32_t* tab, const uint32_t* lstw, uint32_t n, uint32_t ltot, uint32_t shift,
+                      uint32_t* desc, const uint32_t* work, uint32_t* range_start, uint32_t* max_load, uint32_t* clear16);
 void launch_pm_offsets(hipStream_t st, const uint16_t* keys16, const uint32_t* desc, const uint32_t* Tp, uint32_t n,
                        const uint32_t* range_start, uint32_t shift, uint32_t ltot, uint32_t* boff, uint32_t* empty_positions);
 void launch_pm_walk(hipStream_t st, const uint16_t* keys16, const uint16_t* idx16, const uint32_t* desc, const uint32_t* Tp,
                     uint32_t n, const uint32_t* range_start, uint32_t shift, uint32_t ltot, const uint32_t* boff,
                     const uint32_t* selend, unsigned long long* mask, unsigned long long* kept_total, void* scratch,
-                    bool scratch_by_records, uint32_t* amb_count,
+                    bool scratch_by_records,
                     const uint32_t* ev_sev = nullptr, const uint32_t* ev_lastns = nullptr,
                     const uint64_t* d_poff = nullptr, uint32_t n_contigs = 0, uint32_t ell = 0);
-void launch_pm_settle(hipStream_t st, const uint16_t* keys16, const uint16_t* idx16, const uint32_t* desc, const uint32_t* Tp,
-                      uint32_t n, const uint32_t* range_start, uint32_t shift, uint32_t ltot, const void* scratch,
-                      bool scratch_by_records, const uint32_t* amb_count, unsigned long long* mask,
-                      unsigned long long* kept_total);
 
 
 void launch_span_mode_share(hipStream_t st, const uint32_t* starts, const uint32_t* ends, uint32_t n, uint32_t* out );
diff --git a/profiles/summarize_pmc.py b/profiles/summarize_pmc.py
--- a/profiles/summarize_pmc.py
+++ b/profiles/summarize_pmc.py
@@ -15,10 +15,9 @@
     "k_pm_prepare_sort": ("read_4", "write_4"),
     "k_pm_offsets": ("read_8", "write_4"),
     "k_pm_rank_mark": ("read_2", "atomic_or64"),
-    "k_pm_descr": ("read_4", "write_4"),
-    "k_pm_range_table": ("read_4", "write_4"),
+    "k_pm_row_sums": ("read_4", "write_4"),
+    "k_pm_tables": ("read_4", "write_4"),
     "k_pm_walk": ("read_2", "atomic_or64"),
-    "k_pm_settle": ("read_2", "atomic_or64"),
     "k_sweep_pack": ("read_4", "write_16"),
     "k_sweep_uniform_ev": ("read_16", "write_4"),
     "k_sweep_expand": ("read_4", "write_4"),
```
